# rpng/suo_slam

Hardware: AMD Instinct MI355X
Metric: frames/sec (obj-crops/sec) YCB-V 640x480 8-obj; ADD(-S) vs ref (higher is better)
Workload: dtype f32 (2 x fp16 split products)

## Files before the change

### suo_slam_amd/build.py

```python
from __future__ import annotations

import os
import subprocess
import sys

HERE = os.path.dirname(os.path.abspath(__file__))
CSRC = os.path.join(HERE, "csrc")
LIB = os.path.join(HERE, "libsuo_hip.so")
SOURCES = ["capi.hip", "net.hip", "net_weights.hip", "conv.hip", "conv_wino.hip", "conv_wino_x3.hip", "conv_small.hip", "stem_x3.hip", "res_small.hip", "res_small_x3.hip", "gemm_persist.hip", "gemm_bf16x3.hip", "misc.hip", "calibrate.hip", "pnp.hip", "lm.hip", "lm_big.hip", "lm_cam.hip", "lm_cam2.hip", "lm_frame.hip", "lm_frame2.hip", "lm_dist.hip", "pose_cov.hip", "ba_comm.hip", "pnp_api.hip", "ba_stage.hip", "ba_api.hip", "ba_ctx.hip", "ba_drive.hip", "pose_cov_api.hip", "frame_geom.hip", "eval.hip", "eval_bop.hip", "eval_nees.hip", "eval_nees_api.hip", "raster.hip", "eval_vsd.hip", "slam_score.hip", "slam_vote.hip"]
HIPCC = os.environ.get("HIPCC", "/opt/rocm/bin/hipcc")
FLAGS = ["--offload-arch=gfx950", "-O3", "-std=c++17", "-fPIC", "-ffp-contract=off"]


def _stale(target, deps):
    if not os.path.exists(target):
        return True
    t = os.path.getmtime(target)
    return any(os.path.getmtime(d) > t for d in deps)


def build(force: bool = False, verbose: bool = True) -> str:
    srcs = [os.path.join(CSRC, s) for s in SOURCES if os.path.exists(os.path.join(CSRC, s))]
    hdrs = [os.path.join(CSRC, f) for f in os.listdir(CSRC) if f.endswith(".h")]
    hdrs.append(os.path.join(os.path.dirname(HERE), "include", "suo_hip.h"))
    objs = []
    procs = []
    for src in srcs:
        obj = src[:-4] + ".o"
        objs.append(obj)
        deps = [src] + hdrs
        if src.endswith("lm_big.hip"):
            deps.append(os.path.join(CSRC, "lm.hip"))
        if force or _stale(obj, deps):
            cmd = [HIPCC] + FLAGS + ["-c", src, "-o", obj]
            if verbose:
                print(" ".join(cmd), flush=True)
            procs.append((src, subprocess.Popen(cmd)))
    for src, p in procs:
        if p.wait() != 0:
            raise RuntimeError(f"hipcc failed on {src}")
    if force or procs or _stale(LIB, objs):
        cmd = [HIPCC, "--offload-arch=gfx950", "-shared", "-fPIC", "-o", LIB] + objs + ["-ldl"]
        if verbose:
            print(" ".join(cmd), flush=True)
        subprocess.check_call(cmd)
    return LIB


if __name__ == "__main__":
    build(force="--force" in sys.argv)
    print(LIB)
```

### suo_slam_amd/csrc/conv_wino_x3.hip

```cpp
#include <string.h>

#include "bf16x3.h"
#include "f16x2.h"
#include "buffer_ops.h"
#include "suo_internal.h"
#include "tune.h"

namespace suo {

typedef float x_f32x4 __attribute__((ext_vector_type(4)));
typedef float x_f32x16 __attribute__((ext_vector_type(16)));
typedef unsigned x_u32x2 __attribute__((ext_vector_type(2)));
typedef unsigned x_u32x4 __attribute__((ext_vector_type(4)));
typedef __bf16 x_bf16x8 __attribute__((ext_vector_type(8)));
typedef _Float16 x_f16x8 __attribute__((ext_vector_type(8)));

__device__ __forceinline__ x_f32x16 x_mfma32(float a, float b, x_f32x16 c) { return __builtin_amdgcn_mfma_f32_32x32x2f32(a, b, c, 0, 0, 0); }
__device__ __forceinline__ int x_acc_row(int r, int lane) { return (r & 3) + 8 * (r >> 2) + 4 * (lane >> 5); }

__device__ __forceinline__ x_f32x4 x_sub4(x_f32x4 a, x_f32x4 b) { return a - b; }
__device__ __forceinline__ x_f32x4 x_add4(x_f32x4 a, x_f32x4 b) { return a + b; }
__device__ __forceinline__ void x_add16(x_f32x16& z, const x_f32x16& t) { z += t; }
__device__ __forceinline__ void x_sub16(x_f32x16& z, const x_f32x16& t) { z -= t; }

constexpr int X_CK = 16, X_PKH = 20, X_TH = 8, X_TW = 16, X_IH = 10, X_IW = 18, X_NPIX = X_IH * X_IW;

void pack_wino_weight_bf16x3(const float* W, int N, int C, int Np, int Cp, const float* out_scale, uint16_t* out) {
    static const double G[4][3] = {{1, 0, 0}, {0.5, 0.5, 0.5}, {0.5, -0.5, 0.5}, {0, 0, 1}};
    const int NB = Np / 32;
    memset(out, 0, (size_t)Np * Cp * 16 * 3 * sizeof(uint16_t));
    for (int n = 0; n < N; ++n)
        for (int c = 0; c < C; ++c) {
            const float* g = W + ((size_t)n * C + c) * 9;
            const double sc = out_scale ? (double)out_scale[n] : 1.0;
            double Gg[4][3], U[4][4];
            for (int i = 0; i < 4; ++i)
                for (int j = 0; j < 3; ++j) Gg[i][j] = G[i][0] * g[j] + G[i][1] * g[3 + j] + G[i][2] * g[6 + j];
            for (int i = 0; i < 4; ++i)
                for (int j = 0; j < 4; ++j) U[i][j] = (Gg[i][0] * G[j][0] + Gg[i][1] * G[j][1] + Gg[i][2] * G[j][2]) * sc;
            const int chunk = c / X_CK, cc = c % X_CK, nb = n / 32, lane = (cc / 8) * 32 + (n % 32), e = cc % 8;
            for (int comp = 0; comp < 16; ++comp) {
                uint16_t t[3];
                s3_split_host((float)(comp >= 12 ? -U[comp >> 2][comp & 3] : U[comp >> 2][comp & 3]), t);
                for (int p = 0; p < 3; ++p) out[((((size_t)(chunk * 16 + comp) * NB + nb) * 3 + p) * 64 + lane) * 8 + e] = t[p];
            }
        }
}

void pack_tail_weight_bf16x3(const float* W3, int N2, int K, uint16_t* out) {
    const int NB = N2 / 32;
    for (int n = 0; n < N2; ++n)
        for (int k = 0; k < K; ++k) {
            const int ks = k / 16, kk = k % 16, lane = (kk / 8) * 32 + (n % 32), e = kk % 8, nb = n / 32;
            uint16_t t[3];
            s3_split_host(W3[(size_t)n * K + k], t);
            for (int p = 0; p < 3; ++p) out[((((size_t)(ks * NB + nb) * 3 + p) * 64 + lane) * 8) + e] = t[p];
        }
}

void pack_wino_weight_f16x2(const float* W, int N, int C, int Np, int Cp, const float* out_scale, uint16_t* out, float* oscale_out) {
    static const double G[4][3] = {{1, 0, 0}, {0.5, 0.5, 0.5}, {0.5, -0.5, 0.5}, {0, 0, 1}};
    const int NB = Np / 32;
    memset(out, 0, (size_t)Np * Cp * 16 * 2 * sizeof(uint16_t));
    for (int n = 0; n < Np; ++n) oscale_out[n] = ldexpf(1.f, -S2_XSHIFT);
    float* Un = (float*)malloc((size_t)C * 16 * sizeof(float));
    for (int n = 0; n < N; ++n) {
        float mx = 0.f;
        for (int c = 0; c < C; ++c) {
            const float* g = W + ((size_t)n * C + c) * 9;
            const double sc = out_scale ? (double)out_scale[n] : 1.0;
            double Gg[4][3];
            for (int i = 0; i < 4; ++i)
                for (int j = 0; j < 3; ++j) Gg[i][j] = G[i][0] * g[j] + G[i][1] * g[3 + j] + G[i][2] * g[6 + j];
            for (int i = 0; i < 4; ++i)
                for (int j = 0; j < 4; ++j) {
                    const float u = (float)((Gg[i][0] * G[j][0] + Gg[i][1] * G[j][1] + Gg[i][2] * G[j][2]) * sc);
                    Un[c * 16 + i * 4 + j] = i == 3 ? -u : u;
                    mx = fmaxf(mx, fabsf(u));
                }
        }
        const int t = s2_row_shift(mx);
        oscale_out[n] = ldexpf(1.f, -(t + S2_XSHIFT));
        for (int c = 0; c < C; ++c) {
            const int chunk = c / X_CK, cc = c % X_CK, nb = n / 32, lane = (cc / 8) * 32 + (n % 32), e = cc % 8;
            for (int comp = 0; comp < 16; ++comp) {
                uint16_t h[2];
                s2_split_host(ldexpf(Un[c * 16 + comp], t), h);
                for (int p = 0; p < 2; ++p) out[((((size_t)(chunk * 16 + comp) * NB + nb) * 2 + p) * 64 + lane) * 8 + e] = h[p];
            }
        }
    }
    free(Un);
}

void pack_tail_weight_f16x2(const float* W3, int N2, int K, uint16_t* out, float* oscale_out) { pack_gemm_weight_f16x2(W3, N2, K, out, oscale_out); }

template <bool FUSE, bool UP = false, bool TX3 = false, int NT = 4, int NP = 3, bool NEXT = false, bool W8 = false>
__global__ __launch_bounds__(W8 ? 512 : 256) __attribute__((amdgpu_waves_per_eu(2))) void wino3x3_x3_kernel(const ConvArgs a) {
    static_assert(NT == 4 || (NT == 2 && !FUSE), "64-channel form: plain convolution only");
    static_assert(!W8 || (NT == 4 && NP == 2 && !NEXT && (TX3 || !FUSE)), "eight waves: the fp16 form of the 128-channel kernel, without the next block's conv1");
    constexpr int NTHR = W8 ? 512 : 256;
    static_assert(!NEXT || (FUSE && TX3 && NP == 2), "the next block's conv1 rides on the fp16 tail");
    static_assert(NP == 3 || !FUSE || TX3, "the fp16 form's tail runs on the fp16 pipe");
    constexpr int HSZ = X_NPIX * X_PKH;
    constexpr int VROW = 16;
    constexpr int VPL = 16 * 32 * VROW;
    constexpr int VFLOATS = NP * VPL / 2;
    constexpr int TAILF = NP * 8 * (64 * 32 + 32) / 4;
    constexpr int SFLOATS = W8 ? (2 * HSZ + VFLOATS > TAILF + 8 * 32 * 36 ? 2 * HSZ + VFLOATS : TAILF + 8 * 32 * 36) : 2 * HSZ + VFLOATS;
    __shared__ __attribute__((aligned(16))) float S[SFLOATS];
    float (*Hin)[HSZ] = reinterpret_cast<float (*)[HSZ]>(&S[0]);
    uint16_t* V = reinterpret_cast<uint16_t*>(&S[2 * HSZ]);
    const int tid = threadIdx.x, lane = tid & 63;
    const int w = __builtin_amdgcn_readfirstlane(tid >> 6);
    const int tiles_x = (a.OW + X_TW - 1) / X_TW, tiles_y = (a.OH + X_TH - 1) / X_TH;
    int bid = blockIdx.x;
    if ((gridDim.x & 7) == 0) bid = (bid & 7) * (gridDim.x >> 3) + (bid >> 3);
    const int l = bid / (tiles_x * tiles_y);
    bid -= l * tiles_x * tiles_y;
    const int ty0 = bid / tiles_x, tx0 = bid - ty0 * tiles_x;
    const int oy0 = ty0 * X_TH, ox0 = tx0 * X_TW;
    const int iy0 = oy0 - 1, ix0 = ox0 - 1;
    const int nch = a.C / X_CK;
    const float* in_l = a.in + (size_t)l * a.H * a.W * a.C;
    const __amdgpu_buffer_rsrc_t in_srd = make_srd(in_l, (size_t)a.H * a.W * a.C * sizeof(float));
    const __amdgpu_buffer_rsrc_t w_srd = make_srd(a.Wp, (size_t)a.N * a.C * 16 * NP * sizeof(uint16_t));
    const __amdgpu_buffer_rsrc_t out_srd = make_srd(a.out + (size_t)l * a.OH * a.OW * a.N, (size_t)a.OH * a.OW * a.N * sizeof(float));

    constexpr int NF4 = X_NPIX * 4, NLD = (NF4 + NTHR - 1) / NTHR;
    int avoff[NLD];
#pragma unroll
    for (int i = 0; i < NLD; ++i) {
        const int idx = tid + i * NTHR;
        const int pix = idx >> 2, cc = idx & 3;
        const int py = pix / X_IW, px = pix - py * X_IW;
        const int iy = iy0 + py, ix = ix0 + px;
        const bool ok = idx < NF4 && iy >= 0 && iy < a.H && ix >= 0 && ix < a.W;
        avoff[i] = ok ? ((iy * a.W + ix) * a.C + cc * 4) * 4 : BUF_OOB;
    }
    x_f32x4 areg[NLD];
    auto gload = [&](int c) {
#pragma unroll
        for (int i = 0; i < NLD; ++i) areg[i] = buf_load(in_srd, avoff[i], c * X_CK * 4);
    };
    float dmax = 0.f;
    const float xs = NP == 2 ? s2_xscale(a.xscale) : 1.f;
    auto sstore = [&](int buf) {
#pragma unroll
        for (int i = 0; i < NLD; ++i) {
            const int idx = tid + i * NTHR;
            if constexpr (NP == 2) {
                areg[i] *= xs;
                dmax = s2_track(s2_track(dmax, areg[i][0], areg[i][1]), areg[i][2], areg[i][3]);
            }
            if (idx < NF4) *(x_f32x4*)&Hin[buf][(idx >> 2) * X_PKH + (idx & 3) * 4] = areg[i];
        }
    };
    const int wvoff = lane * 16;
    const int wn = NT == 4 ? (W8 ? (w & 3) : w) : (w & 1), wc = NT == 4 ? (W8 ? (w >> 2) : 0) : (w >> 1);
    constexpr bool HALF = NT == 2 || W8;
    constexpr int NPAIR = HALF ? 4 : 8;
    const int wsbase = wn * NP * 1024;
    auto bload = [&](int gc, x_u32x4 (&b)[NP]) {
        const int g = gc;
#pragma unroll
        for (int p = 0; p < NP; ++p) b[p] = __builtin_bit_cast(x_u32x4, buf_load(w_srd, wvoff + p * 1024, g * (NT * NP * 1024) + wsbase));
    };
    const int tt = tid & 31, tq = (tid >> 5) & 3, th = (tid >> 7) & 1;
    const int tv = __builtin_amdgcn_readfirstlane(tid >> 8);
    const int t_ty = tt >> 3, t_tx = tt & 7;
    const int hbase = ((2 * t_ty + th) * X_IW + 2 * t_tx) * X_PKH + tq * 4;
    const int vbase = tt * VROW + ((((tq >> 1) ^ (((tt >> 2) ^ (tt >> 3)) & 1)) * 8) + (tq & 1) * 4);
    auto vstore = [&](int comp, x_f32x4 v) {
        if constexpr (NP == 2) {
            const unsigned h0 = s2_pack_rn(v[0], v[1]), h1 = s2_pack_rn(v[2], v[3]);
            *(x_u32x2*)&V[comp * 32 * VROW + vbase] = x_u32x2{h0, h1};
            const unsigned l0 = s2_lo_pack(v[0], v[1], h0), l1 = s2_lo_pack(v[2], v[3], h1);
            *(x_u32x2*)&V[VPL + comp * 32 * VROW + vbase] = x_u32x2{l0, l1};
            return;
        }
#pragma unroll
        for (int p = 0; p < 3; ++p) {
            const unsigned q0 = s3_pack_rn(v[0], v[1]), q1 = s3_pack_rn(v[2], v[3]);
            *(x_u32x2*)&V[p * VPL + comp * 32 * VROW + vbase] = x_u32x2{q0, q1};
            if (p < 2) {
                v = x_sub4(v, x_f32x4{s3_lo(q0), s3_hi(q0), s3_lo(q1), s3_hi(q1)});
            }
        }
    };
    const int hother = th ? 0 : 2 * X_IW * X_PKH;
    const float hsign = th ? -1.f : 1.f;
    auto transform = [&](int buf) {
        const float* hs = &Hin[buf][hbase];
        if constexpr (W8) {
            const int xi = tv == 0 ? (th ? 3 : 0) : (th ? 2 : 1);
            x_f32x4 e[4];
#pragma unroll
            for (int c = 0; c < 4; ++c) {
                if (tv == 0) {
                    e[c] = x_sub4(*(const x_f32x4*)(hs + c * X_PKH), *(const x_f32x4*)(hs + (2 * X_IW + c) * X_PKH));
                } else {
                    const x_f32x4 l1 = *(const x_f32x4*)(hs + (X_IW + c) * X_PKH), lx = *(const x_f32x4*)(hs + hother + c * X_PKH);
                    e[c] = x_f32x4{__builtin_fmaf(lx[0], hsign, l1[0]), __builtin_fmaf(lx[1], hsign, l1[1]), __builtin_fmaf(lx[2], hsign, l1[2]), __builtin_fmaf(lx[3], hsign, l1[3])};
                }
            }
            vstore(xi * 4 + 0, x_sub4(e[0], e[2]));
            vstore(xi * 4 + 1, x_add4(e[1], e[2]));
            vstore(xi * 4 + 2, x_sub4(e[2], e[1]));
            vstore(xi * 4 + 3, x_sub4(e[1], e[3]));
            return;
        }
        x_f32x4 L0[4], L1[4], L2[4], Lx[4];
#pragma unroll
        for (int c = 0; c < 4; ++c) {
            L0[c] = *(const x_f32x4*)(hs + c * X_PKH);
            L1[c] = *(const x_f32x4*)(hs + (X_IW + c) * X_PKH);
            L2[c] = *(const x_f32x4*)(hs + (2 * X_IW + c) * X_PKH);
            Lx[c] = *(const x_f32x4*)(hs + hother + c * X_PKH);
        }
        x_f32x4 eA[4], eB[4];
#pragma unroll
        for (int c = 0; c < 4; ++c) {
            eA[c] = x_sub4(L0[c], L2[c]);
            eB[c] = x_f32x4{__builtin_fmaf(Lx[c][0], hsign, L1[c][0]), __builtin_fmaf(Lx[c][1], hsign, L1[c][1]), __builtin_fmaf(Lx[c][2], hsign, L1[c][2]),
                            __builtin_fmaf(Lx[c][3], hsign, L1[c][3])};
        }
        const int xiA = th ? 3 : 0, xiB = th ? 2 : 1;
        vstore(xiA * 4 + 0, x_sub4(eA[0], eA[2]));
        vstore(xiA * 4 + 1, x_add4(eA[1], eA[2]));
        vstore(xiA * 4 + 2, x_sub4(eA[2], eA[1]));
        vstore(xiA * 4 + 3, x_sub4(eA[1], eA[3]));
        vstore(xiB * 4 + 0, x_sub4(eB[0], eB[2]));
        vstore(xiB * 4 + 1, x_add4(eB[1], eB[2]));
        vstore(xiB * 4 + 2, x_sub4(eB[2], eB[1]));
        vstore(xiB * 4 + 3, x_sub4(eB[1], eB[3]));
    };

    x_f32x16 zero16;
#pragma unroll
    for (int r = 0; r < 16; ++r) zero16[r] = 0.f;
    x_f32x16 out[4], Z[8];
#pragma unroll
    for (int p = 0; p < 4; ++p)
#pragma unroll
        for (int r = 0; r < 16; ++r) out[p][r] = 0.f;
#pragma unroll
    for (int p = 0; p < 8; ++p)
#pragma unroll
        for (int r = 0; r < 16; ++r) Z[p][r] = 0.f;
    auto mac6 = [&](x_f32x16& acc, const x_bf16x8 (&f)[NP], const x_u32x4 (&bw)[NP], bool from_zero) {
        if constexpr (NP == 2) {
            constexpr int UI[3] = {0, 1, 0}, UJ[3] = {1, 0, 0};
#pragma unroll
            for (int t = 0; t < 3; ++t)
                acc = __builtin_amdgcn_mfma_f32_32x32x16_f16(__builtin_bit_cast(x_f16x8, f[UI[t]]), __builtin_bit_cast(x_f16x8, bw[UJ[t]]), (t == 0 && from_zero) ? zero16 : acc, 0, 0, 0);
            return;
        }
        constexpr int TI[6] = {0, 1, 2, 0, 1, 0}, TJ[6] = {2, 1, 0, 1, 0, 0};
#pragma unroll
        for (int t = 0; t < 6; ++t)
            acc = __builtin_amdgcn_mfma_f32_32x32x16_bf16(f[TI[t] % NP], __builtin_bit_cast(x_bf16x8, bw[TJ[t] % NP]), (t == 0 && from_zero) ? zero16 : acc, 0, 0, 0);
    };
    auto comp_of = [&](int pair, int which) -> int {
        if (!HALF) return pair < 4 ? (which ? 12 + pair : pair) : (which ? 8 + (pair - 4) : 4 + (pair - 4));
        return wc * 8 + 2 * pair + which;
    };
    const int afoff = (lane & 31) * VROW + (((lane >> 5) ^ (((lane >> 2) ^ (lane >> 3)) & 1)) * 8);
    x_u32x4 bring[2][2][NP];
    gload(0);
    bload(comp_of(0, 0), bring[0][0]);
    bload(comp_of(0, 1), bring[0][1]);
    sstore(0);
    __syncthreads();

#ifdef SUO_WX3_PROF
    long long pt[5] = {0, 0, 0, 0, 0}, p0 = clock64();
#define XPROF(i) do { const long long _t = clock64(); pt[i] += _t - p0; p0 = _t; } while (0)
#else
#define XPROF(i) do { } while (0)
#endif
    for (int c = 0; c < nch; ++c) {
        const int buf = c & 1;
        const bool more = c + 1 < nch;
        if (more) gload(c + 1);
        transform(buf);
        XPROF(0);
        __syncthreads();
        XPROF(1);
        if (more) sstore(buf ^ 1);
        XPROF(2);
#pragma unroll
        for (int pair = 0; pair < NPAIR; ++pair) {
            const int slot = pair & 1;
            {
                const int np = pair + 1 < NPAIR ? pair + 1 : 0, nc = pair + 1 < NPAIR ? c : (more ? c + 1 : c);
                bload(nc * 16 + comp_of(np, 0), bring[slot ^ 1][0]);
                bload(nc * 16 + comp_of(np, 1), bring[slot ^ 1][1]);
            }
            const int ca = comp_of(pair, 0), cb = comp_of(pair, 1);
            x_bf16x8 afa[NP], afb[NP];
#pragma unroll
            for (int p = 0; p < NP; ++p) {
                afa[p] = *(const x_bf16x8*)&V[p * VPL + ca * 32 * VROW + afoff];
                afb[p] = *(const x_bf16x8*)&V[p * VPL + cb * 32 * VROW + afoff];
            }
            __builtin_amdgcn_sched_barrier(0);
            if (HALF) {
                mac6(Z[2 * pair], afa, bring[slot][0], false);
                mac6(Z[2 * pair + 1], afb, bring[slot][1], false);
            } else if (pair < 4) {
                mac6(Z[pair], afa, bring[slot][0], false);
                mac6(Z[4 + pair], afb, bring[slot][1], false);
            } else {
                x_f32x16 ta, tb;
                mac6(ta, afa, bring[slot][0], true);
                mac6(tb, afb, bring[slot][1], true);
                x_add16(Z[pair - 4], ta); x_add16(Z[pair - 4], tb); x_add16(Z[pair], ta); x_sub16(Z[pair], tb);
            }
            __builtin_amdgcn_sched_barrier(0);
        }
        XPROF(3);
        __syncthreads();
        XPROF(4);
    }
#ifdef SUO_WX3_PROF
    if (blockIdx.x == 1000 && (tid & 63) == 0) printf("wave %d cycles: transform %lld  barrier1 %lld  sstore %lld  mfma+fold %lld  barrier2 %lld\n", w, pt[0], pt[1], pt[2], pt[3], pt[4]);
#endif
    if constexpr (NP == 2) s2_raise(a.range_flag, 4.f * dmax);
#pragma unroll
    for (int h = 0; h < 2; ++h) {
        out[2 * h] = Z[4 * h] + Z[4 * h + 1] + Z[4 * h + 2];
        out[2 * h + 1] = Z[4 * h + 1] - Z[4 * h + 2] - Z[4 * h + 3];
    }
    x_f32x16 mine[2];
    if constexpr (W8) {
        static_assert(VFLOATS >= 8 * 16 * 64, "the exchange area is the V planes");
        float* X = &S[2 * HSZ];
        const int pw = (1 - wc) * 4 + wn;
#pragma unroll
        for (int q = 0; q < 2; ++q) {
#pragma unroll
            for (int r = 0; r < 16; ++r) X[(w * 16 + r) * 64 + lane] = wc == 0 ? out[2 + q][r] : out[q][r];
            __syncthreads();
#pragma unroll
            for (int r = 0; r < 16; ++r) mine[q][r] = (wc == 0 ? out[q][r] + out[2 + q][r] : out[2 + q][r] - out[q][r]) + X[(pw * 16 + r) * 64 + lane];
            __syncthreads();
        }
    }

    if constexpr (FUSE && TX3) {
        constexpr int KS_STRIDE = 64 * 32 + 32;
        constexpr int PL_STRIDE = 8 * KS_STRIDE;
        static_assert(NP * PL_STRIDE == TAILF * 4 && NP * PL_STRIDE + (W8 ? 8 : 4) * 32 * 36 * 4 <= SFLOATS * 4, "tail staging must fit the workgroup's LDS");
        constexpr int NJ = W8 ? 1 : 2;
        unsigned char* AP = reinterpret_cast<unsigned char*>(&S[0]);
        float* T = &S[NP * PL_STRIDE / 4] + w * (32 * 36);
        const __amdgpu_buffer_rsrc_t w3_srd = make_srd(a.W3p, (size_t)a.N * a.N2 * NP * sizeof(uint16_t));
        const size_t crop2 = (size_t)a.OH * a.OW * a.N2;
        const __amdgpu_buffer_rsrc_t r_srd = make_srd(a.R + (size_t)l * crop2, crop2 * sizeof(float));
        const __amdgpu_buffer_rsrc_t o2_srd = make_srd(a.out2 + (size_t)l * crop2, crop2 * sizeof(float));
        constexpr bool has_up = UP;
        const __amdgpu_buffer_rsrc_t up_srd = make_srd(has_up ? a.up + (size_t)l * (crop2 / 4) : a.R, has_up ? crop2 / 4 * sizeof(float) : 0);
        const float xs3 = NP == 2 ? s2_xscale(a.xscale3) : 1.f;
        const float b2v = NP == 2 ? a.bias[wn * 32 + (lane & 31)] * xs3 : a.bias[wn * 32 + (lane & 31)];
        const float c2v = NP == 2 ? a.oscale[wn * 32 + (lane & 31)] * xs3 : 1.f;
        float tmax = 0.f;
        const int sbase = (2 * wn + ((lane >> 4) & 1)) * KS_STRIDE + (lane >> 5) * (8 * 32) + ((((lane >> 3) & 1) ^ (lane >> 5)) * 16) + (lane & 7) * 2;
        const int aoff = (lane & 31) * 32 + (((lane >> 5) ^ ((lane >> 3) & 1)) * 16);
        const int w3voff = lane * 16;
        auto b3load = [&](int ks, x_u32x4 (&b)[2][NP]) {
            const int k = ks < 8 ? ks : 7;
#pragma unroll
            for (int j = 0; j < NJ; ++j)
#pragma unroll
                for (int p = 0; p < NP; ++p) b[j][p] = __builtin_bit_cast(x_u32x4, buf_load(w3_srd, w3voff, (((k * 8 + (W8 ? w : 4 * j + w)) * NP) + p) * 1024));
        };
#pragma unroll
        for (int h = 0; h < 2; ++h) {
            x_u32x4 b3[2][2][NP];
            b3load(0, b3[0]);
            if (!W8 || wc == h)
#pragma unroll
            for (int pj = 0; pj < 2; ++pj)
#pragma unroll
                for (int r = 0; r < 16; ++r) {
                    const float cv = W8 ? mine[pj][r] : out[2 * h + pj][r];
                    float v = NP == 2 ? fmaxf(fmaf(cv, c2v, b2v), 0.f) : fmaxf(cv + b2v, 0.f);
                    const int off = sbase + (16 * (r >> 2) + 2 * (r & 3) + pj) * 32;
                    if constexpr (NP == 2) {
                        tmax = fmaxf(tmax, v);
                        const _Float16 hi = (_Float16)v, lo = (_Float16)(v - (float)hi);
                        *reinterpret_cast<_Float16*>(AP + off) = hi;
                        *reinterpret_cast<_Float16*>(AP + PL_STRIDE + off) = lo;
                        continue;
                    }
#pragma unroll
                    for (int p = 0; p < 3; ++p) {
                        const unsigned q = s3_pack_rn(v, v);
                        *reinterpret_cast<uint16_t*>(AP + p * PL_STRIDE + off) = (uint16_t)(q >> 16);
                        if (p < 2) v -= s3_hi(q);
                    }
                }
            __syncthreads();
            x_f32x16 acc2[2][2];
#pragma unroll
            for (int i = 0; i < 2; ++i)
#pragma unroll
                for (int j = 0; j < 2; ++j)
#pragma unroll
                    for (int r = 0; r < 16; ++r) acc2[i][j][r] = 0.f;
#pragma unroll
            for (int ks = 0; ks < 8; ++ks) {
                b3load(ks + 1, b3[(ks + 1) & 1]);
                x_bf16x8 af[2][NP];
#pragma unroll
                for (int i = 0; i < 2; ++i)
#pragma unroll
                    for (int p = 0; p < NP; ++p) af[i][p] = *(const x_bf16x8*)(AP + p * PL_STRIDE + ks * KS_STRIDE + i * 1024 + aoff);
                __builtin_amdgcn_sched_barrier(0);
#pragma unroll
                for (int i = 0; i < 2; ++i)
#pragma unroll
                    for (int j = 0; j < NJ; ++j) mac6(acc2[i][j], af[i], b3[ks & 1][j], false);
                __builtin_amdgcn_sched_barrier(0);
            }
            if constexpr (NEXT) __syncthreads();
            x_f32x16 acc1[2];
            if constexpr (NEXT) {
#pragma unroll
                for (int i = 0; i < 2; ++i) acc1[i] = zero16;
            }
#pragma unroll
            for (int j = 0; j < NJ; ++j) {
#pragma unroll
                for (int i = 0; i < 2; ++i) {
                    const int col = (W8 ? w : 4 * j + w) * 32 + (lane & 7) * 4;
                    const x_f32x4 bv = *(const x_f32x4*)(a.bias3 + col);
                    x_f32x4 osc3 = x_f32x4{1.f, 1.f, 1.f, 1.f};
                    if constexpr (NP == 2) osc3 = *(const x_f32x4*)(a.oscale3 + col);
                    x_f32x4 nsc, nsh;
                    if constexpr (NEXT) { const float nxs = s2_xscale(a.n_xscale); nsc = *(const x_f32x4*)(a.n_scale + col) * nxs; nsh = *(const x_f32x4*)(a.n_shift + col) * nxs; }
                    int off[4];
                    x_f32x4 rv[4], uv[UP ? 4 : 1];
#pragma unroll
                    for (int k = 0; k < 4; ++k) {
                        const int m = 32 * i + (lane >> 3) + 8 * k;
                        const int oy = oy0 + 2 * (m >> 4) + h, ox = ox0 + (m & 15);
                        const bool in = oy < a.OH && ox < a.OW;
                        off[k] = in ? ((oy * a.OW + ox) * a.N2 + col) * 4 : BUF_OOB;
                        rv[k] = buf_load(r_srd, off[k], 0);
                        if constexpr (UP && !NEXT) uv[k] = buf_load(up_srd, in ? (((oy >> 1) * (a.OW >> 1) + (ox >> 1)) * a.N2 + col) * 4 : BUF_OOB, 0);
                    }
#pragma unroll
                    for (int r = 0; r < 16; ++r) T[x_acc_row(r, lane) * 36 + (lane & 31)] = acc2[i][j][r];
                    __builtin_amdgcn_wave_barrier();
#pragma unroll
                    for (int k = 0; k < 4; ++k) {
                        if constexpr (UP && NEXT) {
                            const int m = 32 * i + (lane >> 3) + 8 * k;
                            const int oy = oy0 + 2 * (m >> 4) + h, ox = ox0 + (m & 15);
                            uv[0] = buf_load(up_srd, (oy < a.OH && ox < a.OW) ? (((oy >> 1) * (a.OW >> 1) + (ox >> 1)) * a.N2 + col) * 4 : BUF_OOB, 0);
                        }
                        x_f32x4 o = *(const x_f32x4*)&T[((lane >> 3) + 8 * k) * 36 + (lane & 7) * 4];
                        if constexpr (NP == 2) o *= osc3;
                        o = (o + bv) + rv[k];
                        if constexpr (UP) o += uv[NEXT ? 0 : k];
                        buf_store(o, o2_srd, off[k]);
                        if constexpr (NEXT) {
                            const int m = 32 * i + (lane >> 3) + 8 * k;
                            float xn[4];
#pragma unroll
                            for (int c = 0; c < 4; ++c) xn[c] = fmaxf(fmaf(o[c], nsc[c], nsh[c]), 0.f);
                            tmax = fmaxf(fmaxf(tmax, fmaxf(xn[0], xn[1])), fmaxf(xn[2], xn[3]));
                            const unsigned h0 = s2_pack_rn(xn[0], xn[1]), h1 = s2_pack_rn(xn[2], xn[3]);
                            const unsigned l0 = s2_lo_pack(xn[0], xn[1], h0), l1 = s2_lo_pack(xn[2], xn[3], h1);
                            unsigned char* d = AP + (2 * w + ((lane & 7) >> 2)) * KS_STRIDE + m * 32 + (((((lane & 3) >> 1) ^ ((m >> 3) & 1))) * 16) + (lane & 1) * 8;
                            *reinterpret_cast<x_u32x2*>(d) = x_u32x2{h0, h1};
                            *reinterpret_cast<x_u32x2*>(d + PL_STRIDE) = x_u32x2{l0, l1};
                        }
                    }
                    __builtin_amdgcn_wave_barrier();
                }
                if constexpr (NEXT) {
                    const __amdgpu_buffer_rsrc_t n1_srd = make_srd(a.n_W1, (size_t)128 * 256 * 2 * sizeof(uint16_t));
                    auto n1load = [&](int q, x_u32x4 (&b)[2]) {
                        const int ksg = 8 * j + (q < 8 ? q : 7);
#pragma unroll
                        for (int p = 0; p < 2; ++p) b[p] = __builtin_bit_cast(x_u32x4, buf_load(n1_srd, w3voff + p * 1024, ((ksg * 4 + w) * 2) * 1024));
                    };
                    constexpr int NR = 4;
                    x_u32x4 nb[NR][2];
#pragma unroll
                    for (int q = 0; q < NR - 1; ++q) n1load(q, nb[q]);
                    __syncthreads();
#pragma unroll
                    for (int q = 0; q < 8; ++q) {
                        n1load(q + NR - 1, nb[(q + NR - 1) % NR]);
                        x_bf16x8 af[2][2];
#pragma unroll
                        for (int i = 0; i < 2; ++i)
#pragma unroll
                            for (int p = 0; p < 2; ++p) af[i][p] = *(const x_bf16x8*)(AP + p * PL_STRIDE + q * KS_STRIDE + i * 1024 + aoff);
                        __builtin_amdgcn_sched_barrier(0);
#pragma unroll
                        for (int i = 0; i < 2; ++i) mac6(acc1[i], af[i], nb[q % NR], false);
                        __builtin_amdgcn_sched_barrier(0);
                    }
                    __syncthreads();
                }
            }
            if constexpr (NEXT) {
                const int col = w * 32 + (lane & 7) * 4;
                const x_f32x4 b1 = *(const x_f32x4*)(a.n_b1 + col), o1 = *(const x_f32x4*)(a.n_osc1 + col);
                const size_t cropn = (size_t)a.OH * a.OW * 128;
                const __amdgpu_buffer_rsrc_t n_srd = make_srd(a.n_out + (size_t)l * cropn, cropn * sizeof(float));
#pragma unroll
                for (int i = 0; i < 2; ++i) {
#pragma unroll
                    for (int r = 0; r < 16; ++r) T[x_acc_row(r, lane) * 36 + (lane & 31)] = acc1[i][r];
                    __builtin_amdgcn_wave_barrier();
#pragma unroll
                    for (int k = 0; k < 4; ++k) {
                        const int m = 32 * i + (lane >> 3) + 8 * k;
                        const int oy = oy0 + 2 * (m >> 4) + h, ox = ox0 + (m & 15);
                        x_f32x4 o = *(const x_f32x4*)&T[((lane >> 3) + 8 * k) * 36 + (lane & 7) * 4];
                        o *= o1;
                        o += b1;
#pragma unroll
                        for (int c = 0; c < 4; ++c) o[c] = fmaxf(o[c], 0.f);
                        buf_store(o, n_srd, (oy < a.OH && ox < a.OW) ? ((oy * a.OW + ox) * 128 + col) * 4 : BUF_OOB);
                    }
                    __builtin_amdgcn_wave_barrier();
                }
            }
            if (h == 0 && !NEXT) __syncthreads();
        }
        if constexpr (NP == 2) s2_raise(a.range_flag, tmax);
        return;
    }

    if constexpr (FUSE && !TX3) {
        constexpr int MP = 132;
        static_assert(128 * MP <= 2 * HSZ + VFLOATS, "the conv2 tile must fit the workgroup's LDS");
        float* M2 = &S[0];
        const int wm = w >> 1, wn = w & 1;
        const int NB2 = a.N2 >> 5;
        const __amdgpu_buffer_rsrc_t w3_srd = make_srd(a.W3p, (size_t)a.N * a.N2 * sizeof(float));
        const size_t crop2 = (size_t)a.OH * a.OW * a.N2;
        const __amdgpu_buffer_rsrc_t r_srd = make_srd(a.R + (size_t)l * crop2, crop2 * sizeof(float));
        const __amdgpu_buffer_rsrc_t o2_srd = make_srd(a.out2 + (size_t)l * crop2, crop2 * sizeof(float));
        constexpr bool has_up = UP;
        const __amdgpu_buffer_rsrc_t up_srd = make_srd(has_up ? a.up + (size_t)l * (crop2 / 4) : a.R, has_up ? crop2 / 4 * sizeof(float) : 0);
        const float b2v = a.bias[w * 32 + (lane & 31)];
        const int w3voff = lane * 16;
        auto b3load = [&](int q, x_f32x4(&b)[4]) {
            const int kg = q < 16 ? q : 15;
#pragma unroll
            for (int j = 0; j < 4; ++j) b[j] = buf_load(w3_srd, w3voff, (kg * NB2 + wn * 4 + j) * 1024);
        };
        constexpr int R3 = 3;
        x_f32x4 b3[R3][4];
#pragma unroll
        for (int r = 0; r < R3 - 1; ++r) b3load(r, b3[r]);
#pragma unroll
        for (int p = 0; p < 4; ++p)
#pragma unroll
            for (int r = 0; r < 16; ++r) {
                const int t = x_acc_row(r, lane);
                const int pix = (2 * (t >> 3) + (p >> 1)) * X_TW + 2 * (t & 7) + (p & 1);
                M2[pix * MP + w * 32 + (lane & 31)] = fmaxf(out[p][r] + b2v, 0.f);
            }
        __syncthreads();
        x_f32x16 acc2[2][4];
#pragma unroll
        for (int i = 0; i < 2; ++i)
#pragma unroll
            for (int j = 0; j < 4; ++j)
#pragma unroll
                for (int r = 0; r < 16; ++r) acc2[i][j][r] = 0.f;
        const float* ms = M2 + ((wm * 2) * 32 + (lane & 31)) * MP + (lane >> 5) * 4;
#pragma unroll
        for (int q = 0; q < 16; ++q) {
            b3load(q + R3 - 1, b3[(q + R3 - 1) % R3]);
            __builtin_amdgcn_sched_barrier(0);
            x_f32x4 af[2];
#pragma unroll
            for (int i = 0; i < 2; ++i) af[i] = *(const x_f32x4*)(ms + i * 32 * MP + q * 8);
#pragma unroll
            for (int t = 0; t < 4; ++t)
#pragma unroll
                for (int i = 0; i < 2; ++i)
#pragma unroll
                    for (int j = 0; j < 4; ++j) acc2[i][j] = x_mfma32(af[i][t], b3[q % R3][j][t], acc2[i][j]);
            __builtin_amdgcn_sched_barrier(0);
        }
        __syncthreads();
#pragma unroll
        for (int i = 0; i < 2; ++i)
#pragma unroll
            for (int j = 0; j < 4; ++j) {
                float* T = M2 + w * (32 * 36);
                const int col = (wn * 4 + j) * 32 + (lane & 7) * 4;
                const x_f32x4 bv = *(const x_f32x4*)(a.bias3 + col);
                int off[4];
                x_f32x4 rv[4], uv[UP ? 4 : 1];
#pragma unroll
                for (int k = 0; k < 4; ++k) {
                    const int pp = (wm * 2 + i) * 32 + (lane >> 3) + 8 * k;
                    const int oy = oy0 + pp / X_TW, ox = ox0 + pp % X_TW;
                    const bool in = oy < a.OH && ox < a.OW;
                    off[k] = in ? ((oy * a.OW + ox) * a.N2 + col) * 4 : BUF_OOB;
                    rv[k] = buf_load(r_srd, off[k], 0);
                    if constexpr (UP) uv[k] = buf_load(up_srd, in ? (((oy >> 1) * (a.OW >> 1) + (ox >> 1)) * a.N2 + col) * 4 : BUF_OOB, 0);
                }
#pragma unroll
                for (int r = 0; r < 16; ++r) T[x_acc_row(r, lane) * 36 + (lane & 31)] = acc2[i][j][r];
                __builtin_amdgcn_wave_barrier();
#pragma unroll
                for (int k = 0; k < 4; ++k) {
                    x_f32x4 o = (*(const x_f32x4*)&T[((lane >> 3) + 8 * k) * 36 + (lane & 7) * 4] + bv) + rv[k];
                    if constexpr (UP) o += uv[k];
                    buf_store(o, o2_srd, off[k]);
                }
                __builtin_amdgcn_wave_barrier();
            }
        return;
    }

    if constexpr (NT == 2 || W8) {
        if constexpr (NT == 2) {
            float* X = &S[2 * HSZ];
#pragma unroll
            for (int q = 0; q < 2; ++q)
#pragma unroll
                for (int r = 0; r < 16; ++r) X[((w * 2 + q) * 16 + r) * 64 + lane] = wc == 0 ? out[2 + q][r] : out[q][r];
            __syncthreads();
            const int pw = (1 - wc) * 2 + wn;
#pragma unroll
            for (int q = 0; q < 2; ++q)
#pragma unroll
                for (int r = 0; r < 16; ++r)
                    mine[q][r] = (wc == 0 ? out[q][r] + out[2 + q][r] : out[2 + q][r] - out[q][r]) + X[((pw * 2 + q) * 16 + r) * 64 + lane];
            __syncthreads();
        }
        float* T = &S[2 * HSZ] + w * (32 * 36);
        const int col = wn * 32 + (lane & 7) * 4;
        const x_f32x4 bv = *(const x_f32x4*)(a.bias + col);
        x_f32x4 osc = x_f32x4{1.f, 1.f, 1.f, 1.f};
        if constexpr (NP == 2) osc = *(const x_f32x4*)(a.oscale + col);
#pragma unroll
        for (int q = 0; q < 2; ++q) {
            const int p = 2 * wc + q, pi = p >> 1, pj = p & 1;
#pragma unroll
            for (int r = 0; r < 16; ++r) T[x_acc_row(r, lane) * 36 + (lane & 31)] = mine[q][r];
            __builtin_amdgcn_wave_barrier();
#pragma unroll
            for (int k = 0; k < 4; ++k) {
                const int t = (lane >> 3) + 8 * k;
                const int oy = oy0 + 2 * (t >> 3) + pi, ox = ox0 + 2 * (t & 7) + pj;
                x_f32x4 o = *(const x_f32x4*)&T[t * 36 + (lane & 7) * 4];
                if constexpr (NP == 2) o *= osc;
                o += bv;
                if (a.relu) {
#pragma unroll
                    for (int z = 0; z < 4; ++z) o[z] = fmaxf(o[z], 0.f);
                }
                buf_store(o, out_srd, (oy < a.OH && ox < a.OW) ? ((oy * a.OW + ox) * a.N + col) * 4 : BUF_OOB);
            }
            __builtin_amdgcn_wave_barrier();
        }
        return;
    }

    float* T = &S[2 * HSZ] + w * (32 * 36);
    const int col = w * 32 + (lane & 7) * 4;
    const x_f32x4 bv = *(const x_f32x4*)(a.bias + col);
    x_f32x4 osc = x_f32x4{1.f, 1.f, 1.f, 1.f};
    if constexpr (NP == 2) osc = *(const x_f32x4*)(a.oscale + col);
#pragma unroll
    for (int p = 0; p < 4; ++p) {
        const int pi = p >> 1, pj = p & 1;
#pragma unroll
        for (int r = 0; r < 16; ++r) T[x_acc_row(r, lane) * 36 + (lane & 31)] = out[p][r];
        __builtin_amdgcn_wave_barrier();
#pragma unroll
        for (int k = 0; k < 4; ++k) {
            const int t = (lane >> 3) + 8 * k;
            const int oy = oy0 + 2 * (t >> 3) + pi, ox = ox0 + 2 * (t & 7) + pj;
            x_f32x4 o = *(const x_f32x4*)&T[t * 36 + (lane & 7) * 4];
            if constexpr (NP == 2) o *= osc;
            o += bv;
            if (a.relu) {
#pragma unroll
                for (int q = 0; q < 4; ++q) o[q] = fmaxf(o[q], 0.f);
            }
            buf_store(o, out_srd, (oy < a.OH && ox < a.OW) ? ((oy * a.OW + ox) * a.N + col) * 4 : BUF_OOB);
        }
        __builtin_amdgcn_wave_barrier();
    }
}

bool conv3x3_wino_f16x2_w8(long tiles) {
    static const long upto = SUO_TUNE("SUO_WINO_W8_TILES", 256);
    return tiles > 0 && tiles <= upto && env_switch("SUO_WINO_W8", 1) != 0;
}

template <int NP>
static int launch_wino_split(const ConvArgs& a, hipStream_t s) {
    if (NP == 2 && (!a.oscale || !a.range_flag)) { suo_set_error("conv3x3_wino_f16x2: oscale / range_flag missing"); return SUO_ERR_ARG; }
    if (a.OH == a.H && a.OW == a.W && a.N == 64 && a.C == 64) {
        const int tiles64 = ((a.OW + X_TW - 1) / X_TW) * ((a.OH + X_TH - 1) / X_TH) * a.L;
        hipLaunchKernelGGL((wino3x3_x3_kernel<false, false, false, 2, NP>), dim3(tiles64), dim3(256), 0, s, a);
        SUO_HIP_CHECK(hipGetLastError());
        return SUO_OK;
    }
    if (a.OH != a.H || a.OW != a.W || a.N != 128 || a.C != 128) {
        suo_set_error("conv3x3_wino_x3: unsupported shape H=%d W=%d C=%d N=%d", a.H, a.W, a.C, a.N);
        return SUO_ERR_ARG;
    }
    const int tiles = ((a.OW + X_TW - 1) / X_TW) * ((a.OH + X_TH - 1) / X_TH) * a.L;
    if (NP == 2 && conv3x3_wino_f16x2_w8(tiles)) hipLaunchKernelGGL((wino3x3_x3_kernel<false, false, false, 4, 2, false, true>), dim3(tiles), dim3(512), 0, s, a);
    else hipLaunchKernelGGL((wino3x3_x3_kernel<false, false, false, 4, NP>), dim3(tiles), dim3(256), 0, s, a);
    SUO_HIP_CHECK(hipGetLastError());
    return SUO_OK;
}
int launch_conv3x3_wino_x3(const ConvArgs& a, hipStream_t s) { return launch_wino_split<3>(a, s); }
int launch_conv3x3_wino_f16x2(const ConvArgs& a, hipStream_t s) { return launch_wino_split<2>(a, s); }

int launch_conv3x3_wino_f16x2_fused(const ConvArgs& a, hipStream_t s) {
    if (a.OH != a.H || a.OW != a.W || a.N != 128 || a.C != 128 || a.N2 != 256 || !a.W3p || !a.bias3 || !a.R || !a.out2 || !a.oscale || !a.oscale3 || !a.range_flag) {
        suo_set_error("conv3x3_wino_f16x2_fused: unsupported shape C=%d N=%d N2=%d", a.C, a.N, a.N2);
        return SUO_ERR_ARG;
    }
    const int tiles = ((a.OW + X_TW - 1) / X_TW) * ((a.OH + X_TH - 1) / X_TH) * a.L;
    if (a.n_W1) {
        if (!a.n_scale || !a.n_shift || !a.n_osc1 || !a.n_b1 || !a.n_out) { suo_set_error("conv3x3_wino_f16x2_fused: incomplete next-block arguments"); return SUO_ERR_ARG; }
        if (a.up) { suo_set_error("conv3x3_wino_f16x2_fused: the next block's conv1 cannot ride on a tail with an up-sampled addend"); return SUO_ERR_ARG; }
        hipLaunchKernelGGL((wino3x3_x3_kernel<true, false, true, 4, 2, true>), dim3(tiles), dim3(256), 0, s, a);
    } else if (conv3x3_wino_f16x2_w8(tiles)) {
        if (a.up) hipLaunchKernelGGL((wino3x3_x3_kernel<true, true, true, 4, 2, false, true>), dim3(tiles), dim3(512), 0, s, a);
        else hipLaunchKernelGGL((wino3x3_x3_kernel<true, false, true, 4, 2, false, true>), dim3(tiles), dim3(512), 0, s, a);
    } else if (a.up) hipLaunchKernelGGL((wino3x3_x3_kernel<true, true, true, 4, 2>), dim3(tiles), dim3(256), 0, s, a);
    else hipLaunchKernelGGL((wino3x3_x3_kernel<true, false, true, 4, 2>), dim3(tiles), dim3(256), 0, s, a);
    SUO_HIP_CHECK(hipGetLastError());
    return SUO_OK;
}

int launch_conv3x3_wino_x3_fused(const ConvArgs& a, hipStream_t s) {
    if (a.OH != a.H || a.OW != a.W || a.N != 128 || a.C != 128 || a.N2 != 256 || !a.W3p || !a.bias3 || !a.R || !a.out2) {
        suo_set_error("conv3x3_wino_x3_fused: unsupported shape C=%d N=%d N2=%d", a.C, a.N, a.N2);
        return SUO_ERR_ARG;
    }
    const int tiles = ((a.OW + X_TW - 1) / X_TW) * ((a.OH + X_TH - 1) / X_TH) * a.L;
    if (a.w3_bf16x3) {
        if (a.up) hipLaunchKernelGGL((wino3x3_x3_kernel<true, true, true>), dim3(tiles), dim3(256), 0, s, a);
        else hipLaunchKernelGGL((wino3x3_x3_kernel<true, false, true>), dim3(tiles), dim3(256), 0, s, a);
    } else {
        if (a.up) hipLaunchKernelGGL((wino3x3_x3_kernel<true, true, false>), dim3(tiles), dim3(256), 0, s, a);
        else hipLaunchKernelGGL((wino3x3_x3_kernel<true, false, false>), dim3(tiles), dim3(256), 0, s, a);
    }
    SUO_HIP_CHECK(hipGetLastError());
    return SUO_OK;
}

}
```

### suo_slam_amd/csrc/net.h

```cpp
#pragma once
#include <map>
#include <memory>
#include <stdexcept>
#include <string>
#include <utility>
#include <vector>

#include "suo_internal.h"

namespace suo {

struct HostTensor {
    const float* data = nullptr;
    std::vector<int64_t> shape;
    size_t numel = 0;
};

struct PipeW { float* w[3] = {nullptr, nullptr, nullptr}; float* osc = nullptr; };
struct GemmW { PipeW w; float* bias = nullptr; int N = 0, n_valid = 0, K1 = 0, K2 = 0; int site = -1; const float* xs16 = nullptr; };
struct ConvW { float* Wp = nullptr; float* bias = nullptr; int N = 0, C = 0, KS = 0; PipeW wino; int site = -1; const float* xs16 = nullptr; };
struct ResidualW {
    float* pro_scale = nullptr; float* pro_shift = nullptr;
    GemmW c1; ConvW c2; GemmW c3;
    int cin = 0, cout = 0; bool has_skip_conv = false;
    PipeW tail;
    PipeW block[3];
};
struct HourglassW {
    int n = 0;
    ResidualW up1[2], low1[2], low2[2], low3[2];
    std::unique_ptr<HourglassW> inner;
};

void pack_gemm_weight(const float* W, int N, int K, int ldw, int Np, int Kp, float* out);
void pack_conv_weight(const float* W, int N, int C, int KS, int Np, int Cp, int CK, const float* out_scale, float* out);

class Net {
public:
    Net(int n, const char* const* names, const float* const* data, const int64_t* const* shapes, const int* ndims, int max_crops);
    ~Net();
    int forward(const void* img, int fmt, int H, int W, const float* boxes, const int* box_img, int L, const float* priors,
                const float* prior_uv, const uint8_t* prior_mask, float* uv, float* cov,
                float* kp_prob, float* kp_logit, float* logits_out, hipStream_t s);
    int forward_staged(const float* in0_user, int L, float* logits_out, hipStream_t s);
    int prepare(int L, int with_priors, hipStream_t s);
    void set_use_graph(bool v) { use_graph_ = v; }
    int pipe() const { return pipe_; }
    int set_pipe(int p);
    int range_exceeded();
    uint64_t last_call() const { return calls_; }
    int call_range_exceeded(uint64_t call);
    int max_crops() const { return max_crops_; }
    int f16x2_sites() const { return (int)sites_.size(); }
    const char* f16x2_site_name(int i) const { return i >= 0 && i < (int)sites_.size() ? sites_[i].name.c_str() : nullptr; }
    int get_f16x2_shifts(int* out, int n) const;
    int set_f16x2_shifts(const int* s, int n);
    int calibrate(const void* img, int fmt, int H, int W, const float* boxes, const int* box_img, int L, hipStream_t s);
    size_t workspace_bytes() const { return ws_floats_ * sizeof(float); }
    int schedule_bytes(int L, int n_frames, int H, int W, int with_priors, double* out, int* n_launches);
    const HostTensor& T(const std::string& name) const;

private:
    static constexpr int kNumSide = 4, kNumEvents = 32;
    static constexpr int kCallRing = 64, kLiveWord = 0, kStickyWord = 16, kSlotWord = 32;
    int commit_call(hipStream_t s);
    void leave_fp16_form();
    bool own_call_invalid();
    void build_weights(int n, const char* const* names, const float* const* data, const int64_t* const* shapes, const int* ndims);
    float* upload(const std::vector<float>& v);
    template <class Pack3, class Pack2>
    void fill_pipes(PipeW& pw, const float* src, size_t numel, int ncol, Pack3 pack3, Pack2 pack2, bool with_bf16 = true);
    void make_gemm(const std::string& conv, const std::string& bn_after, const std::string& conv2, GemmW& g);
    void pack_gemm(const std::vector<float>& full, const std::vector<float>& bias, int N, int K1, int K2, GemmW& g);
    void make_conv(const std::string& conv, const std::string& bn_after, int CK, ConvW& c, int c_used = 0);
    void make_residual(const std::string& p, ResidualW& r);
    void make_hourglass(const std::string& p, int n, HourglassW& h);
    float* alloc(size_t floats);
    struct BlockPlan {
        enum Route { ONE_LAUNCH,
                     DIRECT_FUSED,
                     WINO_FUSED,
                     PER_LAYER };
        Route route = PER_LAYER;
        bool wino = false;
        int form = 0;
        int form1 = 0, form3 = 0;
        bool takes_up = false;
        bool can_carry_next_conv1 = false;
        bool uses_producer_conv1 = false;
    };
    BlockPlan plan_block(const ResidualW& r, int L, int H, int W) const;
    int residual(const ResidualW& r, const float* x, float* out, int L, int H, int W, hipStream_t s, const float* up = nullptr, float* pool_out = nullptr,
                 const ResidualW* next = nullptr);
    long wino_min_tiles() const;
    long x3_min_rows() const;
    int gemm_form(const GemmW& gw, long M) const;
    int gemm_maybe_pooled(GemmArgs& g, int L, int H, int W, float* pool_out, hipStream_t s, const GemmW& gw, int form);
    int residual_one_launch(const ResidualW& r, const BlockPlan& p, const float* x, float* out, int L, int H, int W, hipStream_t s, const float* up, bool pool_in);
    std::pair<float*, float*> layout_slabs();
    int hourglass(const HourglassW& h, const float* x, float* out, int L, int H, int W, hipStream_t s, int depth_idx, const float* x_pooled = nullptr);
    int backbone(const float* in0, int in_c, float* logits, int L, hipStream_t s, bool stem_done = false);
    int run_backbone(float* in0, int in_c, float* logits, int L, hipStream_t s, bool stem_done = false);
    int ensure_graph(float* in0, int in_c, float* logits, int L, hipStream_t s, hipGraphExec_t* exec, bool stem_done = false);
    bool fused_stem() const;
    int follow_null_stream();

    static constexpr int kMaxSites = 256;
    struct Site {
        std::string name; int ksize = 1; int shift = 4;
        std::vector<std::pair<float*, std::vector<float>>> osc;
    };
    std::vector<Site> sites_;
    float* site_xs_ = nullptr;
    unsigned* probe_max_ = nullptr;
    bool probe_ = false;
    std::vector<char> probed_;
    int add_site(const std::string& name, int ksize);
    void site_osc(int site, float* dev, int n);
    void register_residual_sites(const std::string& p, ResidualW& r);
    void register_gemm_site(const std::string& p, GemmW& g);
    int apply_shifts(const std::vector<int>& s);
    int probe_site(int site, const float* x, long rows, int C, int ld, const float* scale, const float* shift, int relu, hipStream_t s);

    std::map<std::string, HostTensor> tensors_;
    std::vector<float*> owned_;
    ConvW stem_, stem_img_;
    PipeW stem_x3_; float* stem_x3_bias_ = nullptr;
    float* stem_slab_ = nullptr;
    float* stem_mid1_slab_ = nullptr;
    bool stem_computes_r1_conv1() const;
    ResidualW r1_, r4_, r5_, post_[2][2];
    HourglassW hg_[2];
    GemmW lin_[2], head_[2], reinject_;
    float* cls_w_ = nullptr; float* cls_b_ = nullptr;
    int max_crops_;
    float* ws_ = nullptr; size_t ws_floats_ = 0, ws_used_ = 0, ws_mark_ = 0;
    float* d_mean_logit_ = nullptr;
    hipStream_t side_[kNumSide] = {}; hipStream_t own_stream_ = nullptr;
    hipEvent_t ev_[kNumEvents] = {}; int ev_next_ = 0;
    bool use_graph_ = true; bool dry_run_ = false;
    bool acct_on_ = false; double acct_[8] = {}; int acct_launches_ = 0;
    void acct(int kind, double bytes) { if (acct_on_) acct_[kind] += bytes; }
    int maxpool(const float* in, float* out, int L, int H, int W, int C, hipStream_t s);
    struct PreConv1 { const float* x; const ResidualW* r; float* mid1; };
    std::vector<PreConv1> pre_;
    int pipe_ = 1, pipe_built_ = 1;
    unsigned* range_flag_ = nullptr;
    uint64_t calls_ = 0;
    int call_pipe_[kCallRing] = {};
    struct GraphEntry { hipGraph_t graph = nullptr; hipGraphExec_t exec[2] = {nullptr, nullptr}; int next = 0; };
    std::map<int, GraphEntry> graphs_;
};

}
```

### suo_slam_amd/csrc/net.hip

```cpp
#include "net.h"
#include "f16x2.h"

#include <math.h>
#include <stdio.h>
#include <string.h>

#include <algorithm>
#include <string>
#include "tune.h"

namespace suo {

Net::Net(int n, const char* const* names, const float* const* data, const int64_t* const* shapes, const int* ndims, int max_crops)
    : max_crops_(max_crops) {
    build_weights(n, names, data, shapes, ndims);
    const size_t guard_bytes = (size_t)(kSlotWord + kCallRing) * sizeof(unsigned);
    if (hipHostMalloc(reinterpret_cast<void**>(&range_flag_), guard_bytes, hipHostMallocMapped) != hipSuccess) throw std::runtime_error("hipHostMalloc(range flag) failed");
    memset(range_flag_, 0, guard_bytes);

    dry_run_ = true;
    ws_floats_ = (size_t)-1 / sizeof(float) / 2;
    (void)layout_slabs();
    size_t need = 0;
    for (int p = pipe_built_; p >= (pipe_built_ == 0 ? 0 : 1); --p) {
        pipe_ = p;
        if (backbone(nullptr, IN_C, nullptr, max_crops_, nullptr) != SUO_OK) throw std::runtime_error("dry run failed");
        need = std::max(need, ws_used_);
    }
    pipe_ = pipe_built_;
    ws_floats_ = need;
    dry_run_ = false;
    if (hipMalloc(&ws_, ws_floats_ * sizeof(float)) != hipSuccess) throw std::runtime_error("hipMalloc(workspace) failed");
    if (hipMalloc(&d_mean_logit_, (size_t)max_crops_ * NUM_KP * sizeof(float)) != hipSuccess)
        throw std::runtime_error("hipMalloc failed");
    if (hipStreamCreateWithFlags(&own_stream_, hipStreamNonBlocking) != hipSuccess) throw std::runtime_error("hipStreamCreate failed");
    for (int i = 0; i < kNumSide; ++i) {
        if (hipStreamCreateWithFlags(&side_[i], hipStreamNonBlocking) != hipSuccess) throw std::runtime_error("hipStreamCreate failed");
    }
    for (int i = 0; i < kNumEvents; ++i)
        if (hipEventCreateWithFlags(&ev_[i], hipEventDisableTiming) != hipSuccess) throw std::runtime_error("hipEventCreate failed");
}

Net::~Net() {
    for (auto& kv : graphs_) { for (int i = 0; i < 2; ++i) if (kv.second.exec[i]) (void)hipGraphExecDestroy(kv.second.exec[i]); (void)hipGraphDestroy(kv.second.graph); }
    for (float* p : owned_) (void)hipFree(p);
    if (ws_) (void)hipFree(ws_);
    if (d_mean_logit_) (void)hipFree(d_mean_logit_);
    if (range_flag_) (void)hipHostFree(range_flag_);
    for (int i = 0; i < kNumSide; ++i) if (side_[i]) (void)hipStreamDestroy(side_[i]);
    if (own_stream_) (void)hipStreamDestroy(own_stream_);
    for (int i = 0; i < kNumEvents; ++i) if (ev_[i]) (void)hipEventDestroy(ev_[i]);
}

std::pair<float*, float*> Net::layout_slabs() {
    ws_used_ = 0;
    float* in0 = alloc((size_t)max_crops_ * CROP * CROP * IN_C);
    float* logits = alloc((size_t)max_crops_ * NUM_KP * HEAT * HEAT);
    stem_slab_ = alloc((size_t)max_crops_ * 128 * 128 * 64);
    stem_mid1_slab_ = alloc((size_t)max_crops_ * 128 * 128 * 64);
    ws_mark_ = ws_used_;
    return {in0, logits};
}

float* Net::alloc(size_t floats) {
    floats = (floats + 63) & ~(size_t)63;
    if (ws_used_ + floats > ws_floats_) throw std::runtime_error("workspace exhausted");
    float* p = ws_ + ws_used_;
    ws_used_ += floats;
    return p;
}

#define SUO_TRY(x) do { int _r = (x); if (_r != SUO_OK) return _r; } while (0)
#define SUO_LAUNCH(x) do { if (acct_on_) ++acct_launches_; if (!dry_run_) { int _r = (x); if (_r != SUO_OK) return _r; } } while (0)
#define SUO_HIP_LIVE(x) do { if (!dry_run_) SUO_HIP_CHECK(x); } while (0)

enum { ACCT_STAGE = 0, ACCT_CONV3 = 1, ACCT_GEMM = 2, ACCT_BLOCK = 3, ACCT_ELTWISE = 4, ACCT_DECODE = 5, ACCT_KINDS = 6 };
static double gemm_bytes(const GemmArgs& g, double wb) {
    const double M = g.M, nv = g.nchw_hw > 0 ? g.n_valid : g.N;
    double b = 4.0 * M * (g.K1 + g.K2) + (g.R ? 4.0 * M * g.N : 0.0) + wb * (double)g.N * (g.K1 + g.K2);
    if (g.out) b += 4.0 * M * nv;
    if (g.pool_out) b += 4.0 * (M / 4) * g.N;
    return b;
}
static double conv_bytes(const ConvArgs& c, double wb, int taps, bool fused) {
    const double pin = (double)c.L * c.H * c.W, pout = (double)c.L * c.OH * c.OW;
    double b = 4.0 * pin * c.C + wb * (double)c.N * c.C * taps;
    if (!fused) return b + 4.0 * pout * c.N;
    b += 4.0 * pout * c.N2 * 2 + wb * (double)c.N2 * c.N;
    if (c.up) b += 4.0 * (pout / 4) * c.N2;
    if (c.n_out) b += 4.0 * pout * 128 + wb * 128.0 * 256.0;
    return b;
}
static double block_bytes(const ResBlockArgs& a, double wb) {
    const double px = (double)a.L * a.H * a.W;
    return 4.0 * px * 256 * (a.pool_in ? 4 : 1) + 4.0 * px * 256 + (a.up ? 4.0 * (px / 4) * 256 : 0.0) + wb * (256.0 * 128 + 128.0 * 128 * 9 + 128.0 * 256);
}

static double weight_bytes(int form) { return form == 1 ? 6 : 4; }

long Net::wino_min_tiles() const {
    static const long env = (long)SUO_TUNE("SUO_WINO_FUSE_TILES", -1);
    return env >= 0 ? env : (pipe_ == 2 ? 32 : 256);
}
long Net::x3_min_rows() const {
    static const long env = (long)SUO_TUNE("SUO_GEMM_X3_MIN_ROWS", -1);
    return env >= 0 ? env : (pipe_ == 2 ? 4096 : 32768);
}
int Net::gemm_form(const GemmW& gw, long M) const {
    return !gw.w.w[1] || M < x3_min_rows() ? 0 : (pipe_ == 2 && gw.w.w[2] ? 2 : 1);
}

static ConvArgs conv2_args(const ResidualW& r, int L, int H, int W) {
    ConvArgs c2 = {};
    c2.L = L; c2.H = H; c2.W = W; c2.C = r.c2.C; c2.Wp = r.c2.Wp; c2.bias = r.c2.bias; c2.OH = H; c2.OW = W; c2.N = r.c2.N; c2.relu = 1;
    return c2;
}

Net::BlockPlan Net::plan_block(const ResidualW& r, int L, int H, int W) const {
    static const int mode = (int)SUO_TUNE("SUO_RES_FUSED", 2);
    static const long max_tiles = (long)SUO_TUNE("SUO_RES_FUSED_MAX_TILES", 768);
    static const int min_side = (int)SUO_TUNE("SUO_RES_FUSED_MIN_SIDE", 16);
    static const long x3_from_env = (long)SUO_TUNE("SUO_RES_FUSED_X3_FROM", 129);
    static const long f16_from = (long)SUO_TUNE("SUO_RES_FUSED_F16_FROM", 33);
    static const int carry_next = (int)SUO_TUNE("SUO_FUSE_NEXT_CONV1", 1);
    int one = 0;
    if (mode > 0 && r.block[0].w[0] && H <= 32 && W <= 32) {
        const long t32 = (long)L * ((H + 3) / 4) * ((W + 7) / 8);
        const long x3_from = (pipe_ == 2 && r.block[0].w[2] && mode >= 2) ? std::min(f16_from, x3_from_env) : x3_from_env;
        if (mode >= 2 && r.block[0].w[1] && t32 >= x3_from && t32 <= max_tiles) one = 2;
        else if (H >= min_side && W >= min_side && (t32 < x3_from || (mode == 1 && t32 <= max_tiles))) one = 1;
    }
    const ConvArgs c2 = conv2_args(r, L, H, W);
    const long M = (long)L * H * W, tiles = (long)((W + 15) / 16) * ((H + 7) / 8) * L, fuse_tiles = wino_min_tiles();
    const bool tail_shape = !r.has_skip_conv && r.c3.N == 256 && r.c3.n_valid == 256 && r.c3.K1 == 128 && r.cin == 256;
    BlockPlan p;
    p.wino = r.c2.wino.w[0] && conv3x3_wino_pays(c2, pipe_ == 2 ? 32 : -1);
    if (probe_) p.route = BlockPlan::PER_LAYER;
    else if (one) p.route = BlockPlan::ONE_LAUNCH;
    else if (!p.wino && tail_shape && conv3x3_fusable(c2)) p.route = BlockPlan::DIRECT_FUSED;
    else if (p.wino && fuse_tiles > 0 && tiles >= fuse_tiles && tail_shape) p.route = BlockPlan::WINO_FUSED;
    const bool tail = p.route == BlockPlan::WINO_FUSED;
    if (p.route == BlockPlan::ONE_LAUNCH) p.form = one == 2 ? (pipe_ == 2 && r.block[0].w[2] ? 2 : 1) : 0;
    else if (p.wino) p.form = pipe_ == 2 && r.c2.wino.w[2] && (!tail || r.tail.w[2]) ? 2 : (r.c2.wino.w[1] && (!tail || r.tail.w[1]) ? 1 : 0);
    p.form1 = gemm_form(r.c1, M); p.form3 = gemm_form(r.c3, M);
    p.takes_up = p.route == BlockPlan::ONE_LAUNCH || tail;
    p.can_carry_next_conv1 = carry_next && tail && p.form == 2 && !conv3x3_wino_f16x2_w8(tiles);
    const bool from_tail = p.form1 == 2 && r.cin == 256 && r.c1.w.osc && r.c1.N == 128 && r.c1.n_valid == 128 && r.c1.K1 == 256 && r.c1.K2 == 0;
    p.uses_producer_conv1 = p.route != BlockPlan::ONE_LAUNCH && (from_tail || (&r == &r1_ && stem_computes_r1_conv1()));
    return p;
}

static double wino_operands(ConvArgs& c, const ResidualW& r, int form, bool tail, unsigned* range_flag) {
    c.Wp = r.c2.wino.w[form];
    if (tail) { c.W3p = r.tail.w[form]; c.w3_bf16x3 = form == 1; }
    if (form == 2) {
        c.oscale = r.c2.wino.osc; c.range_flag = range_flag; c.xscale = r.c2.xs16;
        if (tail) { c.oscale3 = r.tail.osc; c.xscale3 = r.c3.xs16; }
    }
    return weight_bytes(form);
}
static int launch_wino(const ConvArgs& c, int form, bool tail, hipStream_t s) {
    static int (*const launch[2][3])(const ConvArgs&, hipStream_t) = {{launch_conv3x3_wino, launch_conv3x3_wino_x3, launch_conv3x3_wino_f16x2},
                                                                     {launch_conv3x3_wino_fused, launch_conv3x3_wino_x3_fused, launch_conv3x3_wino_f16x2_fused}};
    return launch[tail][form](c, s);
}

int Net::residual_one_launch(const ResidualW& r, const BlockPlan& p, const float* x, float* out, int L, int H, int W, hipStream_t s, const float* up, bool pool_in) {
    ResBlockArgs a = {};
    a.x = x; a.L = L; a.H = H; a.W = W; a.pool_in = pool_in ? 1 : 0; a.pro_scale = r.pro_scale; a.pro_shift = r.pro_shift;
    a.b1 = r.c1.bias; a.b2 = r.c2.bias; a.b3 = r.c3.bias; a.up = up; a.out = out;
    a.W1 = r.block[0].w[p.form]; a.W2 = r.block[1].w[p.form]; a.W3 = r.block[2].w[p.form];
    if (p.form == 2) {
        a.osc1 = r.block[0].osc; a.osc2 = r.block[1].osc; a.osc3 = r.block[2].osc; a.range_flag = range_flag_;
        a.xs1 = r.c1.xs16; a.xs2 = r.c2.xs16; a.xs3 = r.c3.xs16;
    }
    acct(ACCT_BLOCK, block_bytes(a, weight_bytes(p.form)));
    static int (*const launch[3])(const ResBlockArgs&, hipStream_t) = {launch_res_block, launch_res_block_x3, launch_res_block_f16x2};
    SUO_LAUNCH(launch[p.form](a, s));
    return SUO_OK;
}

int Net::maxpool(const float* in, float* out, int L, int H, int W, int C, hipStream_t s) {
    acct(ACCT_ELTWISE, 4.0 * L * H * W * C * 1.25);
    SUO_LAUNCH(launch_maxpool2(in, out, L, H, W, C, s));
    return SUO_OK;
}

int Net::gemm_maybe_pooled(GemmArgs& g, int L, int H, int W, float* pool_out, hipStream_t s, const GemmW& gw, int form) {
    static const int fuse_pool = (int)suo::env_switch("SUO_FUSE_POOL", 1);
    if (form) {
        GemmArgs gx = g;
        gx.pool_out = pool_out; gx.pool_H = H; gx.pool_W = W;
        if (form == 2) { gx.oscale = gw.w.osc; gx.range_flag = range_flag_; gx.xscale = gw.xs16; }
        auto launch = [&](const GemmArgs& a) { return (form == 2 ? launch_gemm_f16x2_args : launch_gemm_bf16x3_args)(a, reinterpret_cast<const uint16_t*>(gw.w.w[form]), s); };
        const bool pool_in_gemm = gemm_bf16x3_takes(gx);
        if (!pool_in_gemm) gx.pool_out = nullptr;
        if (pool_in_gemm || (g.out && gemm_bf16x3_takes(gx))) {
            acct(ACCT_GEMM, gemm_bytes(gx, weight_bytes(form)));
            SUO_LAUNCH(launch(gx));
            return !pool_in_gemm && pool_out ? maxpool(g.out, pool_out, L, H, W, g.N, s) : SUO_OK;
        }
    }
    if (!pool_out) { acct(ACCT_GEMM, gemm_bytes(g, 4)); SUO_LAUNCH(launch_gemm1x1(g, s)); return SUO_OK; }
    GemmArgs gp = g;
    gp.pool_out = pool_out; gp.pool_H = H; gp.pool_W = W;
    const long tiles128 = (long)(g.M / 128) * (g.N / 128);
    if (fuse_pool && g.M > 4096 && tiles128 >= 512 && gemm1x1_can_pool(gp)) { acct(ACCT_GEMM, gemm_bytes(gp, 4)); SUO_LAUNCH(launch_gemm1x1(gp, s)); return SUO_OK; }
    if (!g.out) g.out = alloc((size_t)g.M * g.ldo);
    acct(ACCT_GEMM, gemm_bytes(g, 4));
    SUO_LAUNCH(launch_gemm1x1(g, s));
    return maxpool(g.out, pool_out, L, H, W, g.N, s);
}

int Net::residual(const ResidualW& r, const float* x, float* out, int L, int H, int W, hipStream_t s, const float* up, float* pool_out, const ResidualW* next) {
    const BlockPlan p = plan_block(r, L, H, W);
    const int M = L * H * W;
    if (up && !p.takes_up) { suo_set_error("residual: an up-sampled addend needs a one-launch block or the fused Winograd tail"); return SUO_ERR_ARG; }
    if (p.route == BlockPlan::ONE_LAUNCH) {
        if (!out) out = alloc((size_t)M * 256);
        SUO_TRY(residual_one_launch(r, p, x, out, L, H, W, s, up, false));
        return pool_out ? maxpool(out, pool_out, L, H, W, 256, s) : SUO_OK;
    }
    float* mid1 = nullptr;
    for (size_t i = 0; p.uses_producer_conv1 && i < pre_.size(); ++i)
        if (pre_[i].x == x && pre_[i].r == &r) {
            mid1 = pre_[i].mid1;
            pre_.erase(pre_.begin() + i);
            break;
        }
    if (!mid1) {
        mid1 = alloc((size_t)M * r.c1.N);
        GemmArgs g1 = {};
        g1.A1 = x; g1.lda1 = r.cin; g1.K1 = r.c1.K1; g1.pro_scale = r.pro_scale; g1.pro_shift = r.pro_shift;
        g1.Wp = r.c1.w.w[0]; g1.bias = r.c1.bias; g1.out = mid1; g1.ldo = r.c1.N; g1.M = M; g1.N = r.c1.N; g1.n_valid = r.c1.n_valid; g1.relu = 1;
        SUO_TRY(gemm_maybe_pooled(g1, L, H, W, nullptr, s, r.c1, p.form1));
    }
    float* mid2 = alloc((size_t)M * r.c2.N);
    ConvArgs c2 = conv2_args(r, L, H, W);
    c2.in = mid1; c2.out = mid2;
    const bool tail = p.route != BlockPlan::PER_LAYER;
    if (tail) {
        if (!out) out = alloc((size_t)M * 256);
        c2.W3p = r.c3.w.w[0]; c2.bias3 = r.c3.bias; c2.R = x; c2.out2 = out; c2.N2 = 256; c2.up = up;
    }
    const double wb = p.wino ? wino_operands(c2, r, p.form, tail, range_flag_) : 4;
    if (next && !up && !pool_out && p.can_carry_next_conv1 && plan_block(*next, L, H, W).uses_producer_conv1) {
        float* nm = alloc((size_t)M * 128);
        c2.n_scale = next->pro_scale; c2.n_shift = next->pro_shift; c2.n_W1 = next->c1.w.w[2]; c2.n_osc1 = next->c1.w.osc; c2.n_b1 = next->c1.bias; c2.n_out = nm; c2.n_xscale = next->c1.xs16;
        pre_.push_back({out, next, nm});
    }
    acct(ACCT_CONV3, conv_bytes(c2, wb, p.wino ? 16 : 9, tail));
    SUO_LAUNCH(p.wino ? launch_wino(c2, p.form, tail, s) : tail ? launch_conv3x3_fused(c2, s) : launch_conv3x3(c2, s));
    if (tail) return pool_out ? maxpool(out, pool_out, L, H, W, 256, s) : SUO_OK;
    GemmArgs g3 = {};
    g3.A1 = mid2; g3.lda1 = r.c2.N; g3.K1 = r.c3.K1;
    if (r.has_skip_conv) { g3.A2 = x; g3.lda2 = r.cin; g3.K2 = r.c3.K2; }
    else { g3.R = x; g3.ldr = r.cin; }
    g3.Wp = r.c3.w.w[0]; g3.bias = r.c3.bias; g3.out = out; g3.ldo = r.cout; g3.M = M; g3.N = r.c3.N; g3.n_valid = r.c3.n_valid;
    if (probe_) {
        SUO_TRY(probe_site(r.c1.site, x, M, r.cin, r.cin, r.pro_scale, r.pro_shift, 1, s));
        SUO_TRY(probe_site(r.c2.site, mid1, M, r.c1.N, r.c1.N, nullptr, nullptr, 0, s));
        SUO_TRY(probe_site(r.c3.site, mid2, M, r.c2.N, r.c2.N, nullptr, nullptr, 0, s));
        if (r.has_skip_conv) SUO_TRY(probe_site(r.c3.site, x, M, r.cin, r.cin, nullptr, nullptr, 0, s));
    }
    return gemm_maybe_pooled(g3, L, H, W, pool_out, s, r.c3, p.form3);
}

int Net::hourglass(const HourglassW& h, const float* x, float* out, int L, int H, int W, hipStream_t s, int depth_idx, const float* x_pooled) {
    const int C = 256;
    const size_t n_hi = (size_t)L * H * W * C, n_lo = n_hi / 4;
    static const int n_side = std::max(0, std::min(kNumSide, (int)env_switch("SUO_NET_SIDE_STREAMS", 0)));
    static const long fork_small = (long)SUO_TUNE("SUO_NET_FORK_SMALL_PIXELS", 0);
    const bool small_fork = !env_set("SUO_SERIAL") && fork_small > 0 && (long)L * H * W <= fork_small && H >= 8;
    const bool serial = (env_set("SUO_SERIAL") || n_side == 0) && !small_fork;
    hipStream_t side = serial ? s : side_[depth_idx % (n_side > 0 ? n_side : kNumSide)];
    hipEvent_t ev_fork = ev_[(ev_next_++) % (kNumEvents - 1)], ev_join = ev_[(ev_next_++) % (kNumEvents - 1)];
    float* up_a = alloc(n_hi);
    float* up_b = alloc(n_hi);
    SUO_HIP_LIVE(hipEventRecord(ev_fork, s));
    SUO_HIP_LIVE(hipStreamWaitEvent(side, ev_fork, 0));
    static const int fuse_up = (int)suo::env_switch("SUO_FUSE_UPSAMPLE", 1);
    const bool up_in_tail = fuse_up && plan_block(h.up1[1], L, H, W).takes_up;
    SUO_TRY(residual(h.up1[0], x, up_a, L, H, W, side, nullptr, nullptr, &h.up1[1]));
    if (!up_in_tail) SUO_TRY(residual(h.up1[1], up_a, up_b, L, H, W, side));
    SUO_HIP_LIVE(hipEventRecord(ev_join, side));

    const float* pooled = x_pooled;
    static const int pool_in_block = (int)SUO_TUNE("SUO_RES_POOL_IN", 1);
    const BlockPlan low1 = plan_block(h.low1[0], L, H / 2, W / 2);
    const bool pool_by_block = !pooled && pool_in_block && low1.route == BlockPlan::ONE_LAUNCH && (H % 2 == 0) && (W % 2 == 0);
    if (!pooled && !pool_by_block) {
        float* p = alloc(n_lo);
        SUO_TRY(maxpool(x, p, L, H, W, C, s));
        pooled = p;
    }
    float* lo_a = alloc(n_lo);
    float* lo_b = alloc(n_lo);
    if (pool_by_block) SUO_TRY(residual_one_launch(h.low1[0], low1, x, lo_a, L, H / 2, W / 2, s, nullptr, true));
    else SUO_TRY(residual(h.low1[0], pooled, lo_a, L, H / 2, W / 2, s, nullptr, nullptr, &h.low1[1]));
    SUO_TRY(residual(h.low1[1], lo_a, lo_b, L, H / 2, W / 2, s, nullptr, nullptr, h.n > 1 ? &h.inner->up1[0] : &h.low2[0]));
    float* low2 = alloc(n_lo);
    if (h.n > 1) {
        SUO_TRY(hourglass(*h.inner, lo_b, low2, L, H / 2, W / 2, s, depth_idx + 1));
    } else {
        float* t = alloc(n_lo);
        SUO_TRY(residual(h.low2[0], lo_b, t, L, H / 2, W / 2, s, nullptr, nullptr, &h.low2[1]));
        SUO_TRY(residual(h.low2[1], t, low2, L, H / 2, W / 2, s, nullptr, nullptr, &h.low3[0]));
    }
    float* l3a = alloc(n_lo);
    float* l3b = alloc(n_lo);
    SUO_TRY(residual(h.low3[0], low2, l3a, L, H / 2, W / 2, s, nullptr, nullptr, &h.low3[1]));
    SUO_TRY(residual(h.low3[1], l3a, l3b, L, H / 2, W / 2, s));
    SUO_HIP_LIVE(hipStreamWaitEvent(s, ev_join, 0));
    if (up_in_tail) SUO_TRY(residual(h.up1[1], up_a, out, L, H, W, s, l3b));
    else { acct(ACCT_ELTWISE, 4.0 * L * H * W * C * 2.25); SUO_LAUNCH(launch_upsample2_add(up_b, l3b, out, L, H, W, C, s)); }
    return SUO_OK;
}

int Net::backbone(const float* in0, int in_c, float* logits, int L, hipStream_t s, bool stem_done) {
    ws_used_ = ws_mark_;
    ev_next_ = 0;
    pre_.clear();
    float* stem = stem_slab_;
    if (stem_done && plan_block(r1_, L, 128, 128).uses_producer_conv1) pre_.push_back({stem, &r1_, stem_mid1_slab_});
    if (!stem_done) {
        ConvArgs c = {};
        const ConvW& sw = in_c == IMG_C ? stem_img_ : stem_;
        c.in = in0; c.L = L; c.H = CROP; c.W = CROP; c.C = in_c; c.Wp = sw.Wp; c.bias = sw.bias;
        c.out = stem; c.OH = 128; c.OW = 128; c.N = 64; c.relu = 1;
        acct(ACCT_STAGE, conv_bytes(c, 4, 49, false));
        SUO_LAUNCH(launch_conv7x7s2(c, s));
    }
    float* p1 = alloc((size_t)L * 64 * 64 * 128);
    SUO_TRY(residual(r1_, stem, nullptr, L, 128, 128, s, nullptr, p1));
    float* r4o = alloc((size_t)L * 64 * 64 * 128);
    SUO_TRY(residual(r4_, p1, r4o, L, 64, 64, s));
    float* x = alloc((size_t)L * 64 * 64 * 256);
    float* xp = alloc((size_t)L * 32 * 32 * 256);
    SUO_TRY(residual(r5_, r4o, x, L, 64, 64, s, nullptr, xp));
    const int M = L * 64 * 64;
    for (int i = 0; i < 2; ++i) {
        float* hg = alloc((size_t)M * 256);
        SUO_TRY(hourglass(hg_[i], x, hg, L, 64, 64, s, 0, xp));
        float* ra = alloc((size_t)M * 256);
        float* rb = alloc((size_t)M * 256);
        SUO_TRY(residual(post_[i][0], hg, ra, L, 64, 64, s, nullptr, nullptr, &post_[i][1]));
        SUO_TRY(residual(post_[i][1], ra, rb, L, 64, 64, s));
        static const int chain_head = (int)SUO_TUNE("SUO_CHAIN_HEAD", 1);
        const long chain_min_rows = x3_min_rows();
        if (i == 1 && chain_head && pipe_ == 2 && lin_[i].w.w[2] && head_[i].w.w[2] && lin_[i].N == 256 && lin_[i].K1 == 256 && M >= chain_min_rows &&
            gemm_chain_head_takes(M, 256, NUM_KP, HEAT * HEAT)) {
            acct(ACCT_GEMM, 4.0 * M * 256 + 4.0 * M * NUM_KP + 4.0 * (256.0 * 256 + 64.0 * 256));
            SUO_LAUNCH(launch_gemm_chain_head(rb, 256, M, reinterpret_cast<const uint16_t*>(lin_[i].w.w[2]), lin_[i].w.osc, lin_[i].bias, reinterpret_cast<const uint16_t*>(head_[i].w.w[2]),
                                              head_[i].w.osc, head_[i].bias, logits, NUM_KP, HEAT * HEAT, range_flag_, s, lin_[i].xs16, head_[i].xs16));
            continue;
        }
        float* ll = alloc((size_t)M * 256);
        GemmArgs gl = {};
        gl.A1 = rb; gl.lda1 = 256; gl.K1 = 256; gl.Wp = lin_[i].w.w[0]; gl.bias = lin_[i].bias; gl.out = ll; gl.ldo = 256;
        gl.M = M; gl.N = 256; gl.n_valid = 256; gl.relu = 1;
        SUO_TRY(gemm_maybe_pooled(gl, L, 64, 64, nullptr, s, lin_[i], gemm_form(lin_[i], M)));
        if (probe_) {
            SUO_TRY(probe_site(lin_[i].site, rb, M, 256, 256, nullptr, nullptr, 0, s));
            SUO_TRY(probe_site(head_[i].site, ll, M, 256, 256, nullptr, nullptr, 0, s));
            if (i == 0) SUO_TRY(probe_site(reinject_.site, ll, M, 256, 256, nullptr, nullptr, 0, s));
        }
        GemmArgs gh = {};
        gh.A1 = ll; gh.lda1 = 256; gh.K1 = 256; gh.Wp = head_[i].w.w[0]; gh.bias = head_[i].bias; gh.M = M; gh.N = 64;
        if (i == 0) {
            float* xn = alloc((size_t)M * 256);
            GemmArgs gr = {};
            gr.A1 = ll; gr.lda1 = 256; gr.K1 = 256;
            gr.Wp = reinject_.w.w[0]; gr.bias = reinject_.bias; gr.R = x; gr.ldr = 256; gr.out = xn; gr.ldo = 256;
            gr.M = M; gr.N = 256; gr.n_valid = 256;
            xp = alloc((size_t)L * 32 * 32 * 256);
            SUO_TRY(gemm_maybe_pooled(gr, L, 64, 64, xp, s, reinject_, gemm_form(reinject_, M)));
            x = xn;
        } else {
            gh.out = logits; gh.n_valid = NUM_KP; gh.nchw_hw = HEAT * HEAT;
            acct(ACCT_GEMM, gemm_bytes(gh, 4));
            SUO_LAUNCH(launch_gemm1x1(gh, s));
        }
    }
    return SUO_OK;
}

int Net::ensure_graph(float* in0, int in_c, float* logits, int L, hipStream_t s, hipGraphExec_t* exec, bool stem_done) {
    const int key = (L * 4 + (in_c == IMG_C ? 1 : 0) + (stem_done ? 2 : 0)) * 4 + pipe_;
    auto it = graphs_.find(key);
    if (it == graphs_.end()) {
        GraphEntry ge;
        SUO_HIP_CHECK(hipStreamBeginCapture(s, hipStreamCaptureModeRelaxed));
        int r;
        try {
            r = backbone(in0, in_c, logits, L, s, stem_done);
        } catch (...) {
            hipGraph_t dead = nullptr;
            (void)hipStreamEndCapture(s, &dead);
            if (dead) (void)hipGraphDestroy(dead);
            throw;
        }
        hipError_t e = hipStreamEndCapture(s, &ge.graph);
        if (r != SUO_OK) return r;
        SUO_HIP_CHECK(e);
        for (int i = 0; i < 2; ++i) SUO_HIP_CHECK(hipGraphInstantiate(&ge.exec[i], ge.graph, nullptr, nullptr, 0));
        it = graphs_.emplace(key, ge).first;
    }
    *exec = it->second.exec[it->second.next];
    it->second.next ^= 1;
    return SUO_OK;
}

int Net::run_backbone(float* in0, int in_c, float* logits, int L, hipStream_t s, bool stem_done) {
    if (use_graph_) {
        hipGraphExec_t exec = nullptr;
        SUO_TRY(ensure_graph(in0, in_c, logits, L, s, &exec, stem_done));
        SUO_HIP_CHECK(hipGraphLaunch(exec, s));
        return SUO_OK;
    }
    return backbone(in0, in_c, logits, L, s, stem_done);
}

int Net::follow_null_stream() {
    hipEvent_t ev = ev_[kNumEvents - 1];
    SUO_HIP_CHECK(hipEventRecord(ev, nullptr));
    SUO_HIP_CHECK(hipStreamWaitEvent(own_stream_, ev, 0));
    return SUO_OK;
}

int Net::set_pipe(int p) {
    if (p < 0 || p > pipe_built_ || (p == 0 && pipe_built_ != 0)) {
        suo_set_error("suo_net_set_pipe: pipe %d not available (this network was built for pipe %d; the fp32 pipe needs SUO_WINO_BF16X3=0 at creation)", p, pipe_built_);
        return SUO_ERR_ARG;
    }
    pipe_ = p;
    return SUO_OK;
}

int Net::get_f16x2_shifts(int* out, int n) const {
    if (!out || n != (int)sites_.size()) { suo_set_error("suo_net_get_f16x2_shifts: %d entries asked, the network has %d sites", n, (int)sites_.size()); return SUO_ERR_ARG; }
    for (int i = 0; i < n; ++i) out[i] = sites_[i].shift;
    return SUO_OK;
}

int Net::apply_shifts(const std::vector<int>& sh) {
    SUO_HIP_CHECK(hipDeviceSynchronize());
    std::vector<float> xs(kMaxSites, S2_XSCALE);
    for (size_t i = 0; i < sites_.size(); ++i) xs[i] = ldexpf(1.f, sh[i]);
    SUO_HIP_CHECK(hipMemcpy(site_xs_, xs.data(), xs.size() * sizeof(float), hipMemcpyHostToDevice));
    for (size_t i = 0; i < sites_.size(); ++i) {
        for (auto& o : sites_[i].osc) {
            std::vector<float> v(o.second.size());
            for (size_t k = 0; k < v.size(); ++k) v[k] = ldexpf(o.second[k], S2_XSHIFT - sh[i]);
            SUO_HIP_CHECK(hipMemcpy(o.first, v.data(), v.size() * sizeof(float), hipMemcpyHostToDevice));
        }
        sites_[i].shift = sh[i];
    }
    if (pipe_built_ == 2) pipe_ = 2;
    return SUO_OK;
}

int Net::set_f16x2_shifts(const int* s, int n) {
    if (sites_.empty()) { suo_set_error("suo_net_set_f16x2_shifts: this network has no fp16 form (built with SUO_F16X2=0 or SUO_WINO_BF16X3=0)"); return SUO_ERR_ARG; }
    if (!s || n != (int)sites_.size()) { suo_set_error("suo_net_set_f16x2_shifts: %d shifts given, the network has %d sites", n, (int)sites_.size()); return SUO_ERR_ARG; }
    for (int i = 0; i < n; ++i)
        if (s[i] < S2_SHIFT_MIN || s[i] > S2_SHIFT_MAX) {
            suo_set_error("suo_net_set_f16x2_shifts: shift %d of site %s outside [%d, %d]", s[i], sites_[i].name.c_str(), S2_SHIFT_MIN, S2_SHIFT_MAX);
            return SUO_ERR_ARG;
        }
    return apply_shifts(std::vector<int>(s, s + n));
}

int Net::probe_site(int site, const float* x, long rows, int C, int ld, const float* scale, const float* shift, int relu, hipStream_t s) {
    if (site < 0) return SUO_OK;
    if (!dry_run_) probed_[site] = 1;
    SUO_LAUNCH(launch_absmax(x, rows, C, ld, scale, shift, relu, probe_max_ + site, s));
    return SUO_OK;
}

int Net::calibrate(const void* img, int fmt, int H, int W, const float* boxes, const int* box_img, int L, hipStream_t s) {
    if (sites_.empty()) { suo_set_error("suo_net_calibrate: this network has no fp16 form (built with SUO_F16X2=0 or SUO_WINO_BF16X3=0)"); return SUO_ERR_ARG; }
    if (L <= 0 || L > max_crops_) { suo_set_error("suo_net_calibrate: L=%d outside [1,%d]", L, max_crops_); return SUO_ERR_ARG; }
    const bool own = (s == nullptr);
    if (own) { s = own_stream_; SUO_TRY(follow_null_stream()); }
    SUO_HIP_CHECK(hipDeviceSynchronize());
    float* const ws = ws_; const size_t ws_floats = ws_floats_, ws_used = ws_used_, ws_mark = ws_mark_;
    float* const stem_slab = stem_slab_; float* const mid1_slab = stem_mid1_slab_;
    const int pipe = pipe_;
    float* pws = nullptr;
    auto restore = [&]() {
        ws_ = ws; ws_floats_ = ws_floats; ws_used_ = ws_used; ws_mark_ = ws_mark; stem_slab_ = stem_slab; stem_mid1_slab_ = mid1_slab;
        pipe_ = pipe; probe_ = false; dry_run_ = false;
        if (pws) { (void)hipStreamSynchronize(s); (void)hipFree(pws); }
    };
    std::vector<unsigned> bits(sites_.size(), 0u);
    auto run = [&]() -> int {
        probe_ = true;
        pipe_ = 1;
        probed_.assign(sites_.size(), 0);
        for (int pass = 0; pass < 2; ++pass) {
            dry_run_ = pass == 0;
            if (pass == 0) ws_floats_ = (size_t)-1 / sizeof(float) / 2;
            else {
                const size_t need = ws_used_;
                SUO_HIP_CHECK(hipMalloc(&pws, need * sizeof(float)));
                ws_ = pws; ws_floats_ = need;
            }
            ws_used_ = 0;
            float* in0 = alloc((size_t)L * CROP * CROP * IN_C);
            float* logits = alloc((size_t)L * NUM_KP * HEAT * HEAT);
            stem_slab_ = alloc((size_t)L * 128 * 128 * 64);
            stem_mid1_slab_ = nullptr;
            ws_mark_ = ws_used_;
            if (pass == 1) {
                SUO_HIP_CHECK(hipMemsetAsync(probe_max_, 0, sites_.size() * sizeof(unsigned), s));
                SUO_TRY(launch_roi_align_concat(img, fmt, H, W, boxes, box_img, L, IMG_C, nullptr, nullptr, nullptr, in0, s));
            }
            SUO_TRY(backbone(in0, IMG_C, logits, L, s, false));
        }
        SUO_HIP_CHECK(hipMemcpyAsync(bits.data(), probe_max_, bits.size() * sizeof(unsigned), hipMemcpyDeviceToHost, s));
        SUO_HIP_CHECK(hipStreamSynchronize(s));
        return SUO_OK;
    };
    int rc;
    try {
        rc = run();
    } catch (const std::exception& e) {
        suo_set_error("suo_net_calibrate: %s", e.what());
        rc = SUO_ERR_ARG;
    }
    restore();
    if (rc != SUO_OK) return rc;
    std::vector<int> sh(sites_.size());
    for (size_t i = 0; i < sites_.size(); ++i) {
        float m;
        memcpy(&m, &bits[i], sizeof(float));
        if (!probed_[i]) { suo_set_error("suo_net_calibrate: the probe did not measure site %s", sites_[i].name.c_str()); return SUO_ERR_ARG; }
        if (!s2_site_shift(m, sites_[i].ksize, &sh[i])) { suo_set_error("suo_net_calibrate: site %s has max |x| = %g", sites_[i].name.c_str(), (double)m); return SUO_ERR_ARG; }
    }
    return apply_shifts(sh);
}

void Net::leave_fp16_form() {
    if (pipe_ != 2) return;
    pipe_ = 1;
    fprintf(stderr, "libsuo_hip: an activation left the fp16 range of its site; this network now runs the three-term bf16 form -- re-issue the call\n");
}

int Net::range_exceeded() {
    const unsigned f = __atomic_exchange_n(range_flag_ + kStickyWord, 0u, __ATOMIC_RELAXED);
    if (!f) return 0;
    leave_fp16_form();
    return 1;
}

static unsigned call_tag(uint64_t call) { return (unsigned)(call & 0x7fffffffu); }

int Net::commit_call(hipStream_t s) {
    const uint64_t c = ++calls_;
    const int i = (int)(c % kCallRing);
    call_pipe_[i] = pipe_;
    if (pipe_ != 2) return SUO_OK;
    return launch_range_commit(range_flag_ + kLiveWord, range_flag_ + kStickyWord, range_flag_ + kSlotWord + i, call_tag(c), s);
}

int Net::call_range_exceeded(uint64_t call) {
    if (call == 0 || call > calls_ || calls_ - call >= (uint64_t)kCallRing) {
        suo_set_error("suo_net_call_range_exceeded: call %llu is not one of the last %d forwards of this network (calls issued: %llu)", (unsigned long long)call,
                      kCallRing, (unsigned long long)calls_);
        return -1;
    }
    const int i = (int)(call % kCallRing);
    if (call_pipe_[i] != 2) return 0;
    const unsigned v = __atomic_load_n(range_flag_ + kSlotWord + i, __ATOMIC_ACQUIRE);
    if ((v >> 1) != call_tag(call)) {
        suo_set_error("suo_net_call_range_exceeded: call %llu has not finished -- synchronise on its outputs first", (unsigned long long)call);
        return -1;
    }
    if (!(v & 1u)) return 0;
    leave_fp16_form();
    return 1;
}

bool Net::own_call_invalid() {
    if (call_range_exceeded(calls_) != 1) return false;
    (void)range_exceeded();
    return true;
}

int Net::schedule_bytes(int L, int n_frames, int H, int W, int with_priors, double* out, int* n_launches) {
    if (L <= 0 || L > max_crops_ || !out) { suo_set_error("suo_net_schedule_bytes: L=%d outside [1,%d] or null output", L, max_crops_); return SUO_ERR_ARG; }
    const bool was_dry = dry_run_;
    dry_run_ = true; acct_on_ = true; acct_launches_ = 0;
    for (int k = 0; k < ACCT_KINDS; ++k) acct_[k] = 0.0;
    int rc = SUO_OK;
    try {
        const double frame_bytes = (double)n_frames * H * W * 3;
        const int in_c = with_priors ? IN_C : IMG_C;
        const bool fstem = !with_priors && fused_stem();
        if (fstem) {
            acct(ACCT_STAGE, frame_bytes + 4.0 * L * 128 * 128 * 64 * (stem_computes_r1_conv1() ? 2 : 1) + 4.0 * 64 * 147);
            ++acct_launches_;
        } else {
            acct(ACCT_STAGE, frame_bytes + 4.0 * L * CROP * CROP * in_c + (with_priors ? 8.0 * L * NUM_KP : 0.0));
            ++acct_launches_;
        }
        rc = backbone(nullptr, in_c, nullptr, L, nullptr, fstem);
        acct(ACCT_DECODE, 4.0 * L * NUM_KP * (HEAT * HEAT + 2 + 4 + 1) + 4.0 * L * NUM_KP * 3 + 4.0 * NUM_KP * (NUM_KP + 1));
        acct_launches_ += 2;
    } catch (const std::exception& e) {
        suo_set_error("suo_net_schedule_bytes: %s", e.what());
        rc = SUO_ERR_ARG;
    }
    dry_run_ = was_dry; acct_on_ = false;
    for (int k = 0; k < ACCT_KINDS; ++k) out[k] = acct_[k];
    if (n_launches) *n_launches = acct_launches_;
    return rc;
}

bool Net::stem_computes_r1_conv1() const {
    static const int on = (int)SUO_TUNE("SUO_STEM_NEXT", 1);
    return on && fused_stem() && pipe_ == 2 && stem_x3_.w[2] && r1_.c1.w.w[2] && r1_.c1.w.osc && r1_.cin == 64 && r1_.c1.N == 64 && r1_.c1.K1 == 64 && r1_.c1.K2 == 0;
}
bool Net::fused_stem() const {
    static const int on = (int)suo::env_switch("SUO_STEM_X3", 1);
    return on != 0 && stem_x3_.w[1] != nullptr;
}

int Net::prepare(int L, int with_priors, hipStream_t s) {
    if (L <= 0 || L > max_crops_) { suo_set_error("suo_net_prepare: L=%d outside [1,%d]", L, max_crops_); return SUO_ERR_ARG; }
    if (!use_graph_) return SUO_OK;
    const bool own = (s == nullptr);
    if (own) s = own_stream_;
    try {
        auto [in0, logits] = layout_slabs();
        hipGraphExec_t exec = nullptr;
        SUO_TRY(ensure_graph(in0, with_priors ? IN_C : IMG_C, logits, L, s, &exec, !with_priors && fused_stem()));
    } catch (const std::exception& e) {
        suo_set_error("suo_net_prepare: %s", e.what());
        return SUO_ERR_ARG;
    }
    return SUO_OK;
}

int Net::forward_staged(const float* in0_user, int L, float* logits_out, hipStream_t s) {
    if (L <= 0 || L > max_crops_) { suo_set_error("suo_net_backbone: L=%d outside [1,%d]", L, max_crops_); return SUO_ERR_ARG; }
    const bool own = (s == nullptr);
    if (own) { s = own_stream_; SUO_TRY(follow_null_stream()); }
    try {
        auto [in0, logits] = layout_slabs();
        if (in0_user)
            SUO_HIP_CHECK(hipMemcpyAsync(in0, in0_user, (size_t)L * CROP * CROP * IN_C * sizeof(float), hipMemcpyDeviceToDevice, s));
        SUO_TRY(run_backbone(in0, IN_C, logits, L, s));
        if (logits_out)
            SUO_HIP_CHECK(hipMemcpyAsync(logits_out, logits, (size_t)L * NUM_KP * HEAT * HEAT * sizeof(float), hipMemcpyDeviceToDevice, s));
        SUO_TRY(commit_call(s));
    } catch (const std::exception& e) {
        suo_set_error("suo_net_backbone: %s", e.what());
        return SUO_ERR_ARG;
    }
    if (own) {
        SUO_HIP_CHECK(hipStreamSynchronize(s));
        if (own_call_invalid()) return forward_staged(in0_user, L, logits_out, nullptr);
    }
    return SUO_OK;
}

int Net::forward(const void* img, int fmt, int H, int W, const float* boxes, const int* box_img, int L, const float* priors,
                 const float* prior_uv, const uint8_t* prior_mask, float* uv, float* cov,
                 float* kp_prob, float* kp_logit, float* logits_out, hipStream_t s) {
    if (L <= 0 || L > max_crops_) { suo_set_error("suo_net_forward: L=%d outside [1,%d]", L, max_crops_); return SUO_ERR_ARG; }
    const bool own = (s == nullptr);
    if (own) { s = own_stream_; SUO_TRY(follow_null_stream()); }
    try {
        auto [in0, logits] = layout_slabs();
        const int in_c = (priors || prior_uv) ? IN_C : IMG_C;
        if (in_c == IMG_C && fused_stem()) {
            const bool f16 = pipe_ == 2 && stem_x3_.w[2];
            const StemNext nx = {r1_.pro_scale, r1_.pro_shift, reinterpret_cast<const uint16_t*>(r1_.c1.w.w[2]), r1_.c1.w.osc, r1_.c1.bias, stem_mid1_slab_, r1_.c1.xs16};
            SUO_LAUNCH(launch_stem_x3(img, fmt, H, W, boxes, box_img, L, reinterpret_cast<const uint16_t*>(stem_x3_.w[f16 ? 2 : 1]), stem_x3_bias_, stem_slab_, s,
                                      f16 ? stem_x3_.osc : nullptr, f16 ? range_flag_ : nullptr, stem_computes_r1_conv1() ? &nx : nullptr));
            SUO_TRY(run_backbone(in0, in_c, logits, L, s, true));
        } else {
            SUO_LAUNCH(launch_roi_align_concat(img, fmt, H, W, boxes, box_img, L, in_c, priors, prior_uv, prior_mask, in0, s));
            SUO_TRY(run_backbone(in0, in_c, logits, L, s, false));
        }
        SUO_LAUNCH(launch_decode(logits, L, uv, cov, d_mean_logit_, nullptr, nullptr, s));
        SUO_LAUNCH(launch_classifier(d_mean_logit_, cls_w_, cls_b_, L, kp_logit, kp_prob, s));
        if (logits_out)
            SUO_HIP_CHECK(hipMemcpyAsync(logits_out, logits, (size_t)L * NUM_KP * HEAT * HEAT * sizeof(float), hipMemcpyDeviceToDevice, s));
        SUO_TRY(commit_call(s));
    } catch (const std::exception& e) {
        suo_set_error("suo_net_forward: %s", e.what());
        return SUO_ERR_ARG;
    }
    if (own) {
        SUO_HIP_CHECK(hipStreamSynchronize(s));
        if (own_call_invalid()) return forward(img, fmt, H, W, boxes, box_img, L, priors, prior_uv, prior_mask, uv, cov, kp_prob, kp_logit, logits_out, nullptr);
    }
    return SUO_OK;
}

}
```

### suo_slam_amd/csrc/suo_internal.h

```cpp
#pragma once
#include <hip/hip_runtime.h>
#include <stdint.h>
#include <stddef.h>

#define SUO_OK 0
#define SUO_ERR_ARG 1
#define SUO_ERR_HIP 2
#define SUO_ERR_MISSING 3

#define SUO_HIP_CHECK(expr)                                                            \
    do {                                                                               \
        hipError_t _e = (expr);                                                        \
        if (_e != hipSuccess) {                                                        \
            suo_set_error("%s:%d %s -> %s", __FILE__, __LINE__, #expr, hipGetErrorString(_e)); \
            return SUO_ERR_HIP;                                                        \
        }                                                                              \
    } while (0)

void suo_set_error(const char* fmt, ...);

namespace suo {

constexpr int NUM_KP = 41;
constexpr int HEAT = 64;
constexpr int CROP = 256;
constexpr int IN_C = 48;
#ifndef SUO_IMG_C
#define SUO_IMG_C 4
#endif
constexpr int IMG_C = SUO_IMG_C;

size_t packed_weight_floats(int n_pad, int k_pad);

struct GemmArgs {
    const float* A1; int lda1; int K1;
    const float* pro_scale; const float* pro_shift;
    const float* A2; int lda2; int K2;
    const float* Wp;
    const float* bias;
    const float* R; int ldr;
    float* out; int ldo;
    int M; int N; int n_valid; int relu; int nchw_hw;
    float* pool_out; int pool_H; int pool_W;
    const float* oscale; unsigned* range_flag;
    const float* xscale;
};
int launch_gemm1x1(const GemmArgs& a, hipStream_t s);
bool gemm1x1_can_pool(const GemmArgs& a);

struct ConvArgs {
    const float* in; int L, H, W, C;
    const float* Wp;
    const float* bias; float* out; int OH, OW, N;
    int relu;
    const float* W3p; const float* bias3; const float* R; float* out2; int N2;
    const float* up;
    int w3_bf16x3;
    const float* oscale; const float* oscale3; unsigned* range_flag;
    const float* n_scale; const float* n_shift; const float* n_W1; const float* n_osc1; const float* n_b1; float* n_out;
    const float* xscale; const float* xscale3; const float* n_xscale;
};
int launch_conv3x3(const ConvArgs& a, hipStream_t s);
bool conv3x3_fusable(const ConvArgs& a);
void pack_wino_weight(const float* W, int N, int C, int Np, int Cp, const float* out_scale, float* out);
int launch_conv3x3_wino(const ConvArgs& a, hipStream_t s);
int launch_conv3x3_wino_fused(const ConvArgs& a, hipStream_t s);
bool conv3x3_wino_pays(const ConvArgs& a, long min_tiles = -1);
int launch_conv3x3_fused(const ConvArgs& a, hipStream_t s);
int launch_conv3x3_small(const ConvArgs& a, hipStream_t s);
int launch_gemm_small(const GemmArgs& a, hipStream_t s);
int launch_gemm_persist(const GemmArgs& a, int cfg, hipStream_t s);
int launch_conv7x7s2(const ConvArgs& a, hipStream_t s);

struct ResBlockArgs {
    const float* x; int L, H, W;
    int pool_in;
    const float* pro_scale; const float* pro_shift;
    const float* W1; const float* b1;
    const float* W2; const float* b2;
    const float* W3; const float* b3;
    const float* up;
    float* out;
    const float* osc1; const float* osc2; const float* osc3; unsigned* range_flag;
    const float* xs1; const float* xs2; const float* xs3;
};
void pack_res16_gemm(const float* W, int N, int K, float* out);
void pack_res16_conv3x3(const float* W, int N, int C, const float* out_scale, float* out);
bool res_block_takes(const ResBlockArgs& a);
int launch_res_block(const ResBlockArgs& a, hipStream_t s);
void pack_res_conv3x3_bf16x3(const float* W, const float* out_scale, uint16_t* out);
int launch_res_block_x3(const ResBlockArgs& a, hipStream_t s);
void pack_res_conv3x3_f16x2(const float* W, const float* out_scale, uint16_t* out, float* oscale_out);
int launch_res_block_f16x2(const ResBlockArgs& a, hipStream_t s);

int launch_maxpool2(const float* in, float* out, int L, int H, int W, int C, hipStream_t s);
int launch_upsample2_add(const float* up1, const float* low, float* out, int L, int H, int W, int C, hipStream_t s);
int launch_roi_align_concat(const void* img, int fmt, int H, int W, const float* boxes, const int* box_img, int L, int out_c,
                            const float* priors, const float* prior_uv, const uint8_t* prior_mask, float* out, hipStream_t s);
int launch_render_priors(const float* uv, const uint8_t* mask, int L, float* out, hipStream_t s);
void pack_gemm_weight_bf16x3(const float* W, int N, int K, uint16_t* out);
bool gemm_bf16x3_takes(const GemmArgs& g);
int launch_gemm_bf16x3_args(const GemmArgs& g, const uint16_t* Wx3, hipStream_t s);
int launch_gemm_bf16x3(const float* A, int lda, int K, const float* pro_scale, const float* pro_shift, const uint16_t* Wp, const float* bias,
                       float* out, int ldo, int M, int N, int relu, hipStream_t s);
void pack_gemm_weight_f16x2(const float* W, int N, int K, uint16_t* out, float* oscale_out);
int launch_gemm_f16x2_args(const GemmArgs& g, const uint16_t* W16, hipStream_t s);
bool gemm_chain_head_takes(int M, int lda, int n_valid, int hw);
int launch_gemm_chain_head(const float* A, int lda, int M, const uint16_t* W1h, const float* osc1, const float* bias1, const uint16_t* W2h, const float* osc2, const float* bias2,
                           float* out, int n_valid, int hw, unsigned* range_flag, hipStream_t s, const float* xs1 = nullptr, const float* xs2 = nullptr);
void pack_tail_weight_bf16x3(const float* W3, int N2, int K, uint16_t* out);
void pack_wino_weight_bf16x3(const float* W, int N, int C, int Np, int Cp, const float* out_scale, uint16_t* out);
int launch_conv3x3_wino_x3(const ConvArgs& a, hipStream_t s);
int launch_conv3x3_wino_x3_fused(const ConvArgs& a, hipStream_t s);
void pack_tail_weight_f16x2(const float* W3, int N2, int K, uint16_t* out, float* oscale_out);
void pack_wino_weight_f16x2(const float* W, int N, int C, int Np, int Cp, const float* out_scale, uint16_t* out, float* oscale_out);
int launch_conv3x3_wino_f16x2(const ConvArgs& a, hipStream_t s);
int launch_conv3x3_wino_f16x2_fused(const ConvArgs& a, hipStream_t s);
bool conv3x3_wino_f16x2_w8(long tiles);
void pack_stem_weight_bf16x3(const float* W, int Cw, const float* out_scale, uint16_t* out);
struct StemNext { const float* scale; const float* shift; const uint16_t* W1; const float* osc1; const float* b1; float* out; const float* xscale = nullptr; };
int launch_stem_x3(const void* img, int fmt, int H, int W, const float* boxes, const int* box_img, int L, const uint16_t* Wx, const float* bias,
                   float* out, hipStream_t s, const float* osc = nullptr, unsigned* range_flag = nullptr, const StemNext* next = nullptr);
void pack_stem_weight_f16x2(const float* W, int Cw, const float* out_scale, uint16_t* out, float* oscale_out);
int launch_upload(void* dst_dev, const void* src_host, size_t bytes, hipStream_t s);
int launch_range_commit(unsigned* live, unsigned* sticky, unsigned* slot, unsigned tag, hipStream_t s);
int launch_absmax(const float* x, long rows, int C, int ld, const float* scale, const float* shift, int relu, unsigned* out, hipStream_t s);
int launch_decode(const float* logits, int L, float* uv, float* cov, float* mean_logit, int* argmax_idx, float* prob, hipStream_t s);
int launch_classifier(const float* mean_logit, const float* Wc, const float* bc, int L,
                      float* kp_logit, float* kp_prob, hipStream_t s);
int launch_kp_masks(const float* uv, const float* cov, const float* kp_prob, const uint8_t* model_mask,
                    int L, float bbox_thresh, float kp_var_thresh, uint8_t* out_mask, hipStream_t s);

}
```

Before: 1366.

## Let next block's conv1 ride on upsample-add Winograd tail behind env switch

Allows the fused Winograd f16x2 tail that adds an up-sampled addend to also compute the following residual block's conv1, passing the next block through hourglass. The aim is to save a separate GEMM launch and a re-read of the hourglass output. The new kernel instantiation is compiled in its own translation unit, and store/load offsets are rewritten with precomputed per-lane column offsets to cut address arithmetic. The fusion is gated by SUO_FUSE_NEXT_CONV1_UP, which defaults to 0, so only the offset rewrite runs by default.

```diff
diff --git a/suo_slam_amd/build.py b/suo_slam_amd/build.py
--- a/suo_slam_amd/build.py
+++ b/suo_slam_amd/build.py
@@ -7,7 +7,7 @@
 HERE = os.path.dirname(os.path.abspath(__file__))
 CSRC = os.path.join(HERE, "csrc")
 LIB = os.path.join(HERE, "libsuo_hip.so")
-SOURCES = ["capi.hip", "net.hip", "net_weights.hip", "conv.hip", "conv_wino.hip", "conv_wino_x3.hip", "conv_small.hip", "stem_x3.hip", "res_small.hip", "res_small_x3.hip", "gemm_persist.hip", "gemm_bf16x3.hip", "misc.hip", "calibrate.hip", "pnp.hip", "lm.hip", "lm_big.hip", "lm_cam.hip", "lm_cam2.hip", "lm_frame.hip", "lm_frame2.hip", "lm_dist.hip", "pose_cov.hip", "ba_comm.hip", "pnp_api.hip", "ba_stage.hip", "ba_api.hip", "ba_ctx.hip", "ba_drive.hip", "pose_cov_api.hip", "frame_geom.hip", "eval.hip", "eval_bop.hip", "eval_nees.hip", "eval_nees_api.hip", "raster.hip", "eval_vsd.hip", "slam_score.hip", "slam_vote.hip"]
+SOURCES = ["capi.hip", "net.hip", "net_weights.hip", "conv.hip", "conv_wino.hip", "conv_wino_x3.hip", "conv_wino_x3_up_next.hip", "conv_small.hip", "stem_x3.hip", "res_small.hip", "res_small_x3.hip", "gemm_persist.hip", "gemm_bf16x3.hip", "misc.hip", "calibrate.hip", "pnp.hip", "lm.hip", "lm_big.hip", "lm_cam.hip", "lm_cam2.hip", "lm_frame.hip", "lm_frame2.hip", "lm_dist.hip", "pose_cov.hip", "ba_comm.hip", "pnp_api.hip", "ba_stage.hip", "ba_api.hip", "ba_ctx.hip", "ba_drive.hip", "pose_cov_api.hip", "frame_geom.hip", "eval.hip", "eval_bop.hip", "eval_nees.hip", "eval_nees_api.hip", "raster.hip", "eval_vsd.hip", "slam_score.hip", "slam_vote.hip"]
 HIPCC = os.environ.get("HIPCC", "/opt/rocm/bin/hipcc")
 FLAGS = ["--offload-arch=gfx950", "-O3", "-std=c++17", "-fPIC", "-ffp-contract=off"]
 
@@ -31,6 +31,8 @@
         deps = [src] + hdrs
         if src.endswith("lm_big.hip"):
             deps.append(os.path.join(CSRC, "lm.hip"))
+        if src.endswith("conv_wino_x3_up_next.hip"):
+            deps.append(os.path.join(CSRC, "conv_wino_x3.hip"))
         if force or _stale(obj, deps):
             cmd = [HIPCC] + FLAGS + ["-c", src, "-o", obj]
             if verbose:
diff --git a/suo_slam_amd/csrc/conv_wino_x3.hip b/suo_slam_amd/csrc/conv_wino_x3.hip
--- a/suo_slam_amd/csrc/conv_wino_x3.hip
+++ b/suo_slam_amd/csrc/conv_wino_x3.hip
@@ -25,6 +25,7 @@
 
 constexpr int X_CK = 16, X_PKH = 20, X_TH = 8, X_TW = 16, X_IH = 10, X_IW = 18, X_NPIX = X_IH * X_IW;
 
+#ifndef SUO_WX3_UP_NEXT_UNIT
 void pack_wino_weight_bf16x3(const float* W, int N, int C, int Np, int Cp, const float* out_scale, uint16_t* out) {
     static const double G[4][3] = {{1, 0, 0}, {0.5, 0.5, 0.5}, {0.5, -0.5, 0.5}, {0, 0, 1}};
     const int NB = Np / 32;
@@ -94,6 +95,7 @@
 }
 
 void pack_tail_weight_f16x2(const float* W3, int N2, int K, uint16_t* out, float* oscale_out) { pack_gemm_weight_f16x2(W3, N2, K, out, oscale_out); }
+#endif
 
 template <bool FUSE, bool UP = false, bool TX3 = false, int NT = 4, int NP = 3, bool NEXT = false, bool W8 = false>
 __global__ __launch_bounds__(W8 ? 512 : 256) __attribute__((amdgpu_waves_per_eu(2))) void wino3x3_x3_kernel(const ConvArgs a) {
@@ -126,6 +128,10 @@
     const __amdgpu_buffer_rsrc_t in_srd = make_srd(in_l, (size_t)a.H * a.W * a.C * sizeof(float));
     const __amdgpu_buffer_rsrc_t w_srd = make_srd(a.Wp, (size_t)a.N * a.C * 16 * NP * sizeof(uint16_t));
     const __amdgpu_buffer_rsrc_t out_srd = make_srd(a.out + (size_t)l * a.OH * a.OW * a.N, (size_t)a.OH * a.OW * a.N * sizeof(float));
+    auto col_voff = [&](int x, int xs, int nc) { return ox0 + x < a.OW ? (xs * nc + (lane & 7) * 4) * 4 : BUF_OOB; };
+    auto row_voff = [&](int oy, int v) { return oy < a.OH ? v : BUF_OOB; };
+    auto st_voff = [&](int oy, int v, int soff) { return oy < a.OH ? v + soff : BUF_OOB; };
+    auto pix_soff = [&](int oy, int ow, int x0, int nc, int ctile) { return ((oy * ow + x0) * nc + ctile * 32) * 4; };
 
     constexpr int NF4 = X_NPIX * 4, NLD = (NF4 + NTHR - 1) / NTHR;
     int avoff[NLD];
@@ -365,6 +371,14 @@
         const float b2v = NP == 2 ? a.bias[wn * 32 + (lane & 31)] * xs3 : a.bias[wn * 32 + (lane & 31)];
         const float c2v = NP == 2 ? a.oscale[wn * 32 + (lane & 31)] * xs3 : 1.f;
         float tmax = 0.f;
+        int vo2[2], vup[2], vn1[2];
+#pragma unroll
+        for (int g = 0; g < 2; ++g) {
+            const int x = (lane >> 3) + 8 * g;
+            vo2[g] = col_voff(x, x, a.N2);
+            if constexpr (UP) vup[g] = col_voff(x, x >> 1, a.N2);
+            if constexpr (NEXT) vn1[g] = col_voff(x, x, 128);
+        }
         const int sbase = (2 * wn + ((lane >> 4) & 1)) * KS_STRIDE + (lane >> 5) * (8 * 32) + ((((lane >> 3) & 1) ^ (lane >> 5)) * 16) + (lane & 7) * 2;
         const int aoff = (lane & 31) * 32 + (((lane >> 5) ^ ((lane >> 3) & 1)) * 16);
         const int w3voff = lane * 16;
@@ -440,32 +454,27 @@
                     if constexpr (NP == 2) osc3 = *(const x_f32x4*)(a.oscale3 + col);
                     x_f32x4 nsc, nsh;
                     if constexpr (NEXT) { const float nxs = s2_xscale(a.n_xscale); nsc = *(const x_f32x4*)(a.n_scale + col) * nxs; nsh = *(const x_f32x4*)(a.n_shift + col) * nxs; }
-                    int off[4];
+                    const int ct = W8 ? w : 4 * j + w;
                     x_f32x4 rv[4], uv[UP ? 4 : 1];
 #pragma unroll
                     for (int k = 0; k < 4; ++k) {
-                        const int m = 32 * i + (lane >> 3) + 8 * k;
-                        const int oy = oy0 + 2 * (m >> 4) + h, ox = ox0 + (m & 15);
-                        const bool in = oy < a.OH && ox < a.OW;
-                        off[k] = in ? ((oy * a.OW + ox) * a.N2 + col) * 4 : BUF_OOB;
-                        rv[k] = buf_load(r_srd, off[k], 0);
-                        if constexpr (UP && !NEXT) uv[k] = buf_load(up_srd, in ? (((oy >> 1) * (a.OW >> 1) + (ox >> 1)) * a.N2 + col) * 4 : BUF_OOB, 0);
+                        const int oy = oy0 + 2 * (2 * i + (k >> 1)) + h;
+                        rv[k] = buf_load(r_srd, row_voff(oy, vo2[k & 1]), pix_soff(oy, a.OW, ox0, a.N2, ct));
+                        if constexpr (UP && !NEXT) uv[k] = buf_load(up_srd, row_voff(oy, vup[k & 1]), pix_soff(oy >> 1, a.OW >> 1, ox0 >> 1, a.N2, ct));
                     }
 #pragma unroll
                     for (int r = 0; r < 16; ++r) T[x_acc_row(r, lane) * 36 + (lane & 31)] = acc2[i][j][r];
                     __builtin_amdgcn_wave_barrier();
 #pragma unroll
                     for (int k = 0; k < 4; ++k) {
-                        if constexpr (UP && NEXT) {
-                            const int m = 32 * i + (lane >> 3) + 8 * k;
-                            const int oy = oy0 + 2 * (m >> 4) + h, ox = ox0 + (m & 15);
-                            uv[0] = buf_load(up_srd, (oy < a.OH && ox < a.OW) ? (((oy >> 1) * (a.OW >> 1) + (ox >> 1)) * a.N2 + col) * 4 : BUF_OOB, 0);
-                        }
+                        const int oy = oy0 + 2 * (2 * i + (k >> 1)) + h;
+                        if constexpr (UP && NEXT)
+                            uv[0] = buf_load(up_srd, row_voff(oy, vup[k & 1]), pix_soff(oy >> 1, a.OW >> 1, ox0 >> 1, a.N2, ct));
                         x_f32x4 o = *(const x_f32x4*)&T[((lane >> 3) + 8 * k) * 36 + (lane & 7) * 4];
                         if constexpr (NP == 2) o *= osc3;
                         o = (o + bv) + rv[k];
                         if constexpr (UP) o += uv[NEXT ? 0 : k];
-                        buf_store(o, o2_srd, off[k]);
+                        buf_store(o, o2_srd, st_voff(oy, vo2[k & 1], pix_soff(oy, a.OW, ox0, a.N2, ct)));
                         if constexpr (NEXT) {
                             const int m = 32 * i + (lane >> 3) + 8 * k;
                             float xn[4];
@@ -521,14 +530,13 @@
                     __builtin_amdgcn_wave_barrier();
 #pragma unroll
                     for (int k = 0; k < 4; ++k) {
-                        const int m = 32 * i + (lane >> 3) + 8 * k;
-                        const int oy = oy0 + 2 * (m >> 4) + h, ox = ox0 + (m & 15);
+                        const int oy = oy0 + 2 * (2 * i + (k >> 1)) + h;
                         x_f32x4 o = *(const x_f32x4*)&T[((lane >> 3) + 8 * k) * 36 + (lane & 7) * 4];
                         o *= o1;
                         o += b1;
 #pragma unroll
                         for (int c = 0; c < 4; ++c) o[c] = fmaxf(o[c], 0.f);
-                        buf_store(o, n_srd, (oy < a.OH && ox < a.OW) ? ((oy * a.OW + ox) * 128 + col) * 4 : BUF_OOB);
+                        buf_store(o, n_srd, st_voff(oy, vn1[k & 1], pix_soff(oy, a.OW, ox0, 128, w)));
                     }
                     __builtin_amdgcn_wave_barrier();
                 }
@@ -595,6 +603,13 @@
             __builtin_amdgcn_sched_barrier(0);
         }
         __syncthreads();
+        int vo2[2], vup[2];
+#pragma unroll
+        for (int g = 0; g < 2; ++g) {
+            const int x = (lane >> 3) + 8 * g;
+            vo2[g] = col_voff(x, x, a.N2);
+            if constexpr (UP) vup[g] = col_voff(x, x >> 1, a.N2);
+        }
 #pragma unroll
         for (int i = 0; i < 2; ++i)
 #pragma unroll
@@ -602,16 +617,12 @@
                 float* T = M2 + w * (32 * 36);
                 const int col = (wn * 4 + j) * 32 + (lane & 7) * 4;
                 const x_f32x4 bv = *(const x_f32x4*)(a.bias3 + col);
-                int off[4];
                 x_f32x4 rv[4], uv[UP ? 4 : 1];
 #pragma unroll
                 for (int k = 0; k < 4; ++k) {
-                    const int pp = (wm * 2 + i) * 32 + (lane >> 3) + 8 * k;
-                    const int oy = oy0 + pp / X_TW, ox = ox0 + pp % X_TW;
-                    const bool in = oy < a.OH && ox < a.OW;
-                    off[k] = in ? ((oy * a.OW + ox) * a.N2 + col) * 4 : BUF_OOB;
-                    rv[k] = buf_load(r_srd, off[k], 0);
-                    if constexpr (UP) uv[k] = buf_load(up_srd, in ? (((oy >> 1) * (a.OW >> 1) + (ox >> 1)) * a.N2 + col) * 4 : BUF_OOB, 0);
+                    const int oy = oy0 + 2 * (wm * 2 + i) + (k >> 1);
+                    rv[k] = buf_load(r_srd, row_voff(oy, vo2[k & 1]), pix_soff(oy, a.OW, ox0, a.N2, wn * 4 + j));
+                    if constexpr (UP) uv[k] = buf_load(up_srd, row_voff(oy, vup[k & 1]), pix_soff(oy >> 1, a.OW >> 1, ox0 >> 1, a.N2, wn * 4 + j));
                 }
 #pragma unroll
                 for (int r = 0; r < 16; ++r) T[x_acc_row(r, lane) * 36 + (lane & 31)] = acc2[i][j][r];
@@ -620,7 +631,8 @@
                 for (int k = 0; k < 4; ++k) {
                     x_f32x4 o = (*(const x_f32x4*)&T[((lane >> 3) + 8 * k) * 36 + (lane & 7) * 4] + bv) + rv[k];
                     if constexpr (UP) o += uv[k];
-                    buf_store(o, o2_srd, off[k]);
+                    const int oy = oy0 + 2 * (wm * 2 + i) + (k >> 1);
+                    buf_store(o, o2_srd, st_voff(oy, vo2[k & 1], pix_soff(oy, a.OW, ox0, a.N2, wn * 4 + j)));
                 }
                 __builtin_amdgcn_wave_barrier();
             }
@@ -648,6 +660,7 @@
         const x_f32x4 bv = *(const x_f32x4*)(a.bias + col);
         x_f32x4 osc = x_f32x4{1.f, 1.f, 1.f, 1.f};
         if constexpr (NP == 2) osc = *(const x_f32x4*)(a.oscale + col);
+        const int vout[2] = {col_voff(2 * (lane >> 3), 2 * (lane >> 3), a.N), col_voff(2 * (lane >> 3) + 1, 2 * (lane >> 3) + 1, a.N)};
 #pragma unroll
         for (int q = 0; q < 2; ++q) {
             const int p = 2 * wc + q, pi = p >> 1, pj = p & 1;
@@ -657,7 +670,7 @@
 #pragma unroll
             for (int k = 0; k < 4; ++k) {
                 const int t = (lane >> 3) + 8 * k;
-                const int oy = oy0 + 2 * (t >> 3) + pi, ox = ox0 + 2 * (t & 7) + pj;
+                const int oy = oy0 + 2 * k + pi;
                 x_f32x4 o = *(const x_f32x4*)&T[t * 36 + (lane & 7) * 4];
                 if constexpr (NP == 2) o *= osc;
                 o += bv;
@@ -665,7 +678,7 @@
 #pragma unroll
                     for (int z = 0; z < 4; ++z) o[z] = fmaxf(o[z], 0.f);
                 }
-                buf_store(o, out_srd, (oy < a.OH && ox < a.OW) ? ((oy * a.OW + ox) * a.N + col) * 4 : BUF_OOB);
+                buf_store(o, out_srd, st_voff(oy, vout[pj], pix_soff(oy, a.OW, ox0, a.N, wn)));
             }
             __builtin_amdgcn_wave_barrier();
         }
@@ -677,6 +690,7 @@
     const x_f32x4 bv = *(const x_f32x4*)(a.bias + col);
     x_f32x4 osc = x_f32x4{1.f, 1.f, 1.f, 1.f};
     if constexpr (NP == 2) osc = *(const x_f32x4*)(a.oscale + col);
+    const int vout[2] = {col_voff(2 * (lane >> 3), 2 * (lane >> 3), a.N), col_voff(2 * (lane >> 3) + 1, 2 * (lane >> 3) + 1, a.N)};
 #pragma unroll
     for (int p = 0; p < 4; ++p) {
         const int pi = p >> 1, pj = p & 1;
@@ -686,7 +700,7 @@
 #pragma unroll
         for (int k = 0; k < 4; ++k) {
             const int t = (lane >> 3) + 8 * k;
-            const int oy = oy0 + 2 * (t >> 3) + pi, ox = ox0 + 2 * (t & 7) + pj;
+            const int oy = oy0 + 2 * k + pi;
             x_f32x4 o = *(const x_f32x4*)&T[t * 36 + (lane & 7) * 4];
             if constexpr (NP == 2) o *= osc;
             o += bv;
@@ -694,16 +708,25 @@
 #pragma unroll
                 for (int q = 0; q < 4; ++q) o[q] = fmaxf(o[q], 0.f);
             }
-            buf_store(o, out_srd, (oy < a.OH && ox < a.OW) ? ((oy * a.OW + ox) * a.N + col) * 4 : BUF_OOB);
+            buf_store(o, out_srd, st_voff(oy, vout[pj], pix_soff(oy, a.OW, ox0, a.N, w)));
         }
         __builtin_amdgcn_wave_barrier();
     }
 }
 
+#ifdef SUO_WX3_UP_NEXT_UNIT
+int launch_conv3x3_wino_f16x2_up_next(const ConvArgs& a, int tiles, hipStream_t s) {
+    hipLaunchKernelGGL((wino3x3_x3_kernel<true, true, true, 4, 2, true>), dim3(tiles), dim3(256), 0, s, a);
+    SUO_HIP_CHECK(hipGetLastError());
+    return SUO_OK;
+}
+#else
 bool conv3x3_wino_f16x2_w8(long tiles) {
     static const long upto = SUO_TUNE("SUO_WINO_W8_TILES", 256);
     return tiles > 0 && tiles <= upto && env_switch("SUO_WINO_W8", 1) != 0;
 }
+
+bool conv3x3_wino_f16x2_tail_next_takes_up(long tiles) { return tiles > 256; }
 
 template <int NP>
 static int launch_wino_split(const ConvArgs& a, hipStream_t s) {
@@ -735,7 +758,11 @@
     const int tiles = ((a.OW + X_TW - 1) / X_TW) * ((a.OH + X_TH - 1) / X_TH) * a.L;
     if (a.n_W1) {
         if (!a.n_scale || !a.n_shift || !a.n_osc1 || !a.n_b1 || !a.n_out) { suo_set_error("conv3x3_wino_f16x2_fused: incomplete next-block arguments"); return SUO_ERR_ARG; }
-        if (a.up) { suo_set_error("conv3x3_wino_f16x2_fused: the next block's conv1 cannot ride on a tail with an up-sampled addend"); return SUO_ERR_ARG; }
+        if (a.up && !conv3x3_wino_f16x2_tail_next_takes_up(tiles)) {
+            suo_set_error("conv3x3_wino_f16x2_fused: the next block's conv1 rides on a tail with an up-sampled addend only in launches of more than 256 tiles (%d)", tiles);
+            return SUO_ERR_ARG;
+        }
+        if (a.up) return launch_conv3x3_wino_f16x2_up_next(a, tiles, s);
         hipLaunchKernelGGL((wino3x3_x3_kernel<true, false, true, 4, 2, true>), dim3(tiles), dim3(256), 0, s, a);
     } else if (conv3x3_wino_f16x2_w8(tiles)) {
         if (a.up) hipLaunchKernelGGL((wino3x3_x3_kernel<true, true, true, 4, 2, false, true>), dim3(tiles), dim3(512), 0, s, a);
@@ -762,5 +789,6 @@
     SUO_HIP_CHECK(hipGetLastError());
     return SUO_OK;
 }
-
-}
+#endif
+
+}
diff --git a/suo_slam_amd/csrc/conv_wino_x3_up_next.hip b/suo_slam_amd/csrc/conv_wino_x3_up_next.hip
--- /dev/null
+++ b/suo_slam_amd/csrc/conv_wino_x3_up_next.hip
@@ -0,0 +1,2 @@
+#define SUO_WX3_UP_NEXT_UNIT 1
+#include "conv_wino_x3.hip"
diff --git a/suo_slam_amd/csrc/net.h b/suo_slam_amd/csrc/net.h
--- a/suo_slam_amd/csrc/net.h
+++ b/suo_slam_amd/csrc/net.h
@@ -87,6 +87,7 @@
         int form1 = 0, form3 = 0;
         bool takes_up = false;
         bool can_carry_next_conv1 = false;
+        bool can_carry_next_conv1_up = false;
         bool uses_producer_conv1 = false;
     };
     BlockPlan plan_block(const ResidualW& r, int L, int H, int W) const;
@@ -98,7 +99,7 @@
     int gemm_maybe_pooled(GemmArgs& g, int L, int H, int W, float* pool_out, hipStream_t s, const GemmW& gw, int form);
     int residual_one_launch(const ResidualW& r, const BlockPlan& p, const float* x, float* out, int L, int H, int W, hipStream_t s, const float* up, bool pool_in);
     std::pair<float*, float*> layout_slabs();
-    int hourglass(const HourglassW& h, const float* x, float* out, int L, int H, int W, hipStream_t s, int depth_idx, const float* x_pooled = nullptr);
+    int hourglass(const HourglassW& h, const float* x, float* out, int L, int H, int W, hipStream_t s, int depth_idx, const ResidualW* next, const float* x_pooled = nullptr);
     int backbone(const float* in0, int in_c, float* logits, int L, hipStream_t s, bool stem_done = false);
     int run_backbone(float* in0, int in_c, float* logits, int L, hipStream_t s, bool stem_done = false);
     int ensure_graph(float* in0, int in_c, float* logits, int L, hipStream_t s, hipGraphExec_t* exec, bool stem_done = false);
diff --git a/suo_slam_amd/csrc/net.hip b/suo_slam_amd/csrc/net.hip
--- a/suo_slam_amd/csrc/net.hip
+++ b/suo_slam_amd/csrc/net.hip
@@ -145,6 +145,8 @@
     p.form1 = gemm_form(r.c1, M); p.form3 = gemm_form(r.c3, M);
     p.takes_up = p.route == BlockPlan::ONE_LAUNCH || tail;
     p.can_carry_next_conv1 = carry_next && tail && p.form == 2 && !conv3x3_wino_f16x2_w8(tiles);
+    const bool carry_next_up = env_switch("SUO_FUSE_NEXT_CONV1_UP", 0) != 0;
+    p.can_carry_next_conv1_up = carry_next_up && p.can_carry_next_conv1 && conv3x3_wino_f16x2_tail_next_takes_up(tiles);
     const bool from_tail = p.form1 == 2 && r.cin == 256 && r.c1.w.osc && r.c1.N == 128 && r.c1.n_valid == 128 && r.c1.K1 == 256 && r.c1.K2 == 0;
     p.uses_producer_conv1 = p.route != BlockPlan::ONE_LAUNCH && (from_tail || (&r == &r1_ && stem_computes_r1_conv1()));
     return p;
@@ -244,7 +246,7 @@
         c2.W3p = r.c3.w.w[0]; c2.bias3 = r.c3.bias; c2.R = x; c2.out2 = out; c2.N2 = 256; c2.up = up;
     }
     const double wb = p.wino ? wino_operands(c2, r, p.form, tail, range_flag_) : 4;
-    if (next && !up && !pool_out && p.can_carry_next_conv1 && plan_block(*next, L, H, W).uses_producer_conv1) {
+    if (next && !pool_out && (up ? p.can_carry_next_conv1_up : p.can_carry_next_conv1) && plan_block(*next, L, H, W).uses_producer_conv1) {
         float* nm = alloc((size_t)M * 128);
         c2.n_scale = next->pro_scale; c2.n_shift = next->pro_shift; c2.n_W1 = next->c1.w.w[2]; c2.n_osc1 = next->c1.w.osc; c2.n_b1 = next->c1.bias; c2.n_out = nm; c2.n_xscale = next->c1.xs16;
         pre_.push_back({out, next, nm});
@@ -266,7 +268,7 @@
     return gemm_maybe_pooled(g3, L, H, W, pool_out, s, r.c3, p.form3);
 }
 
-int Net::hourglass(const HourglassW& h, const float* x, float* out, int L, int H, int W, hipStream_t s, int depth_idx, const float* x_pooled) {
+int Net::hourglass(const HourglassW& h, const float* x, float* out, int L, int H, int W, hipStream_t s, int depth_idx, const ResidualW* next, const float* x_pooled) {
     const int C = 256;
     const size_t n_hi = (size_t)L * H * W * C, n_lo = n_hi / 4;
     static const int n_side = std::max(0, std::min(kNumSide, (int)env_switch("SUO_NET_SIDE_STREAMS", 0)));
@@ -301,7 +303,7 @@
     SUO_TRY(residual(h.low1[1], lo_a, lo_b, L, H / 2, W / 2, s, nullptr, nullptr, h.n > 1 ? &h.inner->up1[0] : &h.low2[0]));
     float* low2 = alloc(n_lo);
     if (h.n > 1) {
-        SUO_TRY(hourglass(*h.inner, lo_b, low2, L, H / 2, W / 2, s, depth_idx + 1));
+        SUO_TRY(hourglass(*h.inner, lo_b, low2, L, H / 2, W / 2, s, depth_idx + 1, &h.low3[0]));
     } else {
         float* t = alloc(n_lo);
         SUO_TRY(residual(h.low2[0], lo_b, t, L, H / 2, W / 2, s, nullptr, nullptr, &h.low2[1]));
@@ -312,7 +314,7 @@
     SUO_TRY(residual(h.low3[0], low2, l3a, L, H / 2, W / 2, s, nullptr, nullptr, &h.low3[1]));
     SUO_TRY(residual(h.low3[1], l3a, l3b, L, H / 2, W / 2, s));
     SUO_HIP_LIVE(hipStreamWaitEvent(s, ev_join, 0));
-    if (up_in_tail) SUO_TRY(residual(h.up1[1], up_a, out, L, H, W, s, l3b));
+    if (up_in_tail) SUO_TRY(residual(h.up1[1], up_a, out, L, H, W, s, l3b, nullptr, next));
     else { acct(ACCT_ELTWISE, 4.0 * L * H * W * C * 2.25); SUO_LAUNCH(launch_upsample2_add(up_b, l3b, out, L, H, W, C, s)); }
     return SUO_OK;
 }
@@ -341,7 +343,7 @@
     const int M = L * 64 * 64;
     for (int i = 0; i < 2; ++i) {
         float* hg = alloc((size_t)M * 256);
-        SUO_TRY(hourglass(hg_[i], x, hg, L, 64, 64, s, 0, xp));
+        SUO_TRY(hourglass(hg_[i], x, hg, L, 64, 64, s, 0, &post_[i][0], xp));
         float* ra = alloc((size_t)M * 256);
         float* rb = alloc((size_t)M * 256);
         SUO_TRY(residual(post_[i][0], hg, ra, L, 64, 64, s, nullptr, nullptr, &post_[i][1]));
diff --git a/suo_slam_amd/csrc/suo_internal.h b/suo_slam_amd/csrc/suo_internal.h
--- a/suo_slam_amd/csrc/suo_internal.h
+++ b/suo_slam_amd/csrc/suo_internal.h
@@ -117,6 +117,8 @@
 int launch_conv3x3_wino_f16x2(const ConvArgs& a, hipStream_t s);
 int launch_conv3x3_wino_f16x2_fused(const ConvArgs& a, hipStream_t s);
 bool conv3x3_wino_f16x2_w8(long tiles);
+int launch_conv3x3_wino_f16x2_up_next(const ConvArgs& a, int tiles, hipStream_t s);
+bool conv3x3_wino_f16x2_tail_next_takes_up(long tiles);
 void pack_stem_weight_bf16x3(const float* W, int Cw, const float* out_scale, uint16_t* out);
 struct StemNext { const float* scale; const float* shift; const uint16_t* W1; const float* osc1; const float* b1; float* out; const float* xscale = nullptr; };
 int launch_stem_x3(const void* img, int fmt, int H, int W, const float* boxes, const int* box_img, int L, const uint16_t* Wx, const float* bias,
```

Result: no change. 1381 (median of 6 runs) (+1.1%).
